# ciccio42/openvla-oft

Measured on AMD Instinct MI355X. Metric: fine-tune samples/s (action-chunks/s) OpenVLA-7B bf16, higher is better.
Workload: dtype bf16; 1 GPU; BASELINE.json configs[2]: LoRA r=32 fine-tune step (fwd+bwd+AdamW), 2x224x224 images + proprio, L1 head; global_batch=8, seq_len=608, parallelism=dp1, mask_mode=bidirectional

## Files before the change

### include/ovla.h

```cpp
#ifndef OVLA_H_
#define OVLA_H_

#include <stdint.h>

#ifdef __cplusplus
extern "C" {
#endif

#define OVLA_OK 0
#define OVLA_EINVAL (-1)
#define OVLA_EARCH (-2)
#define OVLA_ELAUNCH (-3)

#define OVLA_ABI_VERSION 1

const char* ovla_last_error(void);
int ovla_abi_version(void);
const char* ovla_build_hash(void);
int ovla_check_device(int device);

enum { OVLA_ACT_NONE = 0, OVLA_ACT_GELU = 1, OVLA_ACT_RELU = 2, OVLA_ACT_SILU = 3, OVLA_ACT_GELU_TANH = 4,
       OVLA_ACT_SWIGLU = 5 };

typedef struct {
  const void* A; int64_t lda;
  const void* B; int64_t ldb;
  const void* A2; int64_t lda2;
  const void* B2; int64_t ldb2;
  void* C; int64_t ldc;
  void* C_pre;
  const void* bias;
  const void* colscale;
  const void* residual; int64_t ldr;
  const void* film_gamma;
  const void* film_beta;
  int32_t film_rows;
  int32_t M, N, K, K2;
  int32_t k2_group_n;
  int32_t a_group_n;
  int32_t act;
  int32_t split_k;
  int32_t tile;
  float alpha;
  const void* dact_src; int64_t ld_dact;
  int32_t dact_mode, dact_act;
  const void* rope_cos; const void* rope_sin;
  int32_t rope_S, rope_cols;
  float* rowsq_out;
  const float* rowscale_part; int32_t rowscale_slots; float rowscale_eps; float* rowscale_r;
  uint32_t* hybrid_counters; int32_t n_hybrid_counters;
  void* workspace;
  int64_t workspace_bytes;
} ovla_gemm_args;

int ovla_gemm_plan(int32_t M, int32_t N, int32_t K, int32_t K2, int32_t k2_group_n, int64_t workspace_bytes, int32_t* tile,
                   int32_t* full_tiles, int32_t* rem_tiles, int32_t* rem_splits, double* est_seconds);
int ovla_gemm_resolved_tile(const ovla_gemm_args* a, int32_t* tile);
int64_t ovla_gemm_workspace_bytes(int32_t M, int32_t N, int32_t split_k);
int ovla_gemm_bf16(const ovla_gemm_args* a, void* stream);

typedef struct {
  int32_t tile;
  int32_t splits;
} ovla_gemm_schedule;
enum { OVLA_EPI_ROPE = 1,
       OVLA_EPI_ROWSCALE = 2,
       OVLA_EPI_SWIGLU = 4,
       OVLA_EPI_GENERAL = 8,
       OVLA_EPI_ROWSQ = 16     };
int ovla_gemm_fixed_schedule(int32_t N, int32_t K, int32_t K2, int32_t k2_group_n, int32_t epi_flags, ovla_gemm_schedule* out);
int64_t ovla_gemm_fixed_workspace_bytes(int32_t M, int32_t N, const ovla_gemm_schedule* s);
int ovla_gemm_bf16_fixed(const ovla_gemm_args* a, const ovla_gemm_schedule* s, void* stream);

typedef struct {
  const void* X; int64_t ldx;
  const void* Y; int64_t ldy;
  void* C; int64_t ldc;
  int32_t M, P, Q;
  float alpha;
  int32_t out_mode;
  float* W;
} ovla_gemm_tn_args;
int64_t ovla_gemm_tn_workspace_floats(const ovla_gemm_tn_args* a, int32_t group_size);
int ovla_gemm_tn_bf16(const ovla_gemm_tn_args* a, void* stream);
#define OVLA_TN_MAX_GROUP 4
int ovla_gemm_tn_grouped(const ovla_gemm_tn_args* problems, int32_t n, void* stream);

typedef struct {
  void* t; int64_t ld;
  const int32_t* obs_slot;
  const int32_t* obs_slot_host;
  int32_t M, G, n, r, rows_per_obs, n_obs;
} ovla_lora_route_args;
int ovla_lora_route(const ovla_lora_route_args* a, void* stream);

typedef struct {
  const void* src; void* dst;
  const int32_t* obs_slot; const int32_t* obs_slot_host;
  int64_t src_slot_stride;
  int32_t n, rows, dim, rows_per_obs, n_obs, elem_bytes;
} ovla_select_by_slot_args;
int ovla_select_by_slot(const ovla_select_by_slot_args* a, void* stream);

#define OVLA_MAX_SLOTS 4
#define OVLA_FILM_MAX_OBS 64
#define OVLA_FILM_ITEM_COLS 4
typedef struct { const void* W; const void* bias; void* out; int32_t out_f; int32_t item_start; } ovla_film_linear;
typedef struct {
  const void* table;
  const void* table_host;
  const void* avg; int64_t ld_avg;
  const int32_t* obs_slot;
  const int32_t* obs_slot_host;
  int32_t n_linears, n_obs, n, D;
} ovla_film_vectors_args;
int ovla_film_vectors(const ovla_film_vectors_args* a, void* stream);


typedef struct {
  const void* x; int64_t ldx;
  void* out[4];
  uint32_t module[4];
  uint32_t seed_lo, seed_hi, call;
  float p;
  int32_t M, K, G;
} ovla_lora_dropout_apply_args;
int ovla_lora_dropout_apply(const ovla_lora_dropout_apply_args* a, void* stream);

typedef struct {
  const void* x; int64_t ldx;
  const void* A; int64_t lda;
  void* t; int64_t ldt;
  uint32_t module[4];
  uint32_t seed_lo, seed_hi, call;
  float p, alpha;
  int32_t M, K, G, r;
} ovla_lora_dropout_proj_args;
int ovla_lora_dropout_proj(const ovla_lora_dropout_proj_args* a, void* stream);

typedef struct {
  void* dx; int64_t ld;
  const void* dt; int64_t ld_dt;
  const void* AT; int64_t ld_at;
  uint32_t module[4];
  uint32_t seed_lo, seed_hi, call;
  float p;
  int32_t M, K, G, r;
} ovla_lora_dropout_backproj_args;
int ovla_lora_dropout_backproj(const ovla_lora_dropout_backproj_args* a, void* stream);

typedef struct { const void* X; int64_t ldx; float* out; int32_t M, N; } ovla_colsum_args;
int ovla_colsum_bf16(const ovla_colsum_args* a, void* stream);

typedef struct {
  const void* Q; const void* K; const void* V; int64_t q_stride, k_stride, v_stride;
  void* O; int64_t o_stride;
  float* lse;
  const int32_t* kv_len;
  int32_t B, H, S, head_dim;
  int32_t causal;
  float scale;
} ovla_attn_fwd_args;
int ovla_attn_fwd(const ovla_attn_fwd_args* a, void* stream);

typedef struct {
  const void* Q; const void* K; const void* V; int64_t q_stride, k_stride, v_stride;
  const void* O; const void* dO; int64_t o_stride, do_stride;
  const float* lse;
  float* delta;
  void* dQ; void* dK; void* dV; int64_t dq_stride, dk_stride, dv_stride;
  const int32_t* kv_len;
  int32_t B, H, S, head_dim;
  int32_t causal;
  float scale;
  const void* rope_cos;
  const void* rope_sin;
} ovla_attn_bwd_args;
int ovla_attn_bwd(const ovla_attn_bwd_args* a, void* stream);

typedef struct {
  const void* Q; const void* K; int64_t q_stride, k_stride;
  const float* lse;
  const int32_t* kv_len;
  const int32_t* rows;
  float* P;
  float* P_mean;
  int32_t B, H, S, R, head_dim, causal; float scale;
} ovla_attn_probs_args;
int ovla_attn_probs(const ovla_attn_probs_args* a, void* stream);

typedef struct {
  const void* x; void* y; const void* weight; const void* bias;
  float* mean; float* rstd;
  int32_t rows, dim; float eps; int32_t is_rms;
} ovla_norm_fwd_args;
int ovla_norm_fwd(const ovla_norm_fwd_args* a, void* stream);

typedef struct {
  const void* x; const void* dy; const void* weight;
  const float* mean; const float* rstd;
  void* dx; float* dweight; float* dbias;
  int32_t rows, dim; int32_t is_rms; int32_t dx_accum;
} ovla_norm_bwd_args;
int ovla_norm_bwd(const ovla_norm_bwd_args* a, void* stream);

int ovla_rope_table(void* cos_table, void* sin_table, int32_t S, int32_t head_dim, float theta, void* stream);
typedef struct {
  void* qk; int64_t ld; int32_t rows, S, n_heads, head_dim;
  const void* cos_table; const void* sin_table; int32_t inverse;
} ovla_rope_args;
int ovla_rope(const ovla_rope_args* a, void* stream);

typedef struct { const void* gu; void* h; int32_t rows, F; } ovla_swiglu_fwd_args;
int ovla_swiglu_fwd(const ovla_swiglu_fwd_args* a, void* stream);
typedef struct { const void* gu; const void* dh; void* dgu; int32_t rows, F; } ovla_swiglu_bwd_args;
int ovla_swiglu_bwd(const ovla_swiglu_bwd_args* a, void* stream);

typedef struct { const void* z; const void* dh; void* dz; int64_t n; int32_t act; } ovla_act_bwd_args;
int ovla_act_bwd(const ovla_act_bwd_args* a, void* stream);

typedef struct { const void* a; const void* b; void* out; int64_t n; } ovla_add_args;
int ovla_add_bf16(const ovla_add_args* a, void* stream);
typedef struct { const void* x; const void* scale; void* out; int32_t rows, dim; } ovla_colscale_args;
int ovla_colscale_bf16(const ovla_colscale_args* a, void* stream);

typedef struct { const void* pixels; void* out; int64_t ldo; int32_t B, C_total, c0, H, W, patch, n_img, img_cstride; } ovla_im2col_args;
int ovla_im2col(const ovla_im2col_args* a, void* stream);

typedef struct { const void* src; void* dst; int32_t n_img, H, W, out, crop; float crop_scale; float mean[6]; float std[6]; } ovla_image_prep_args;
int ovla_image_prep(const ovla_image_prep_args* a, void* stream);

typedef struct {
  const void* src; void* dst; void* workspace; int64_t workspace_bytes;
  const int32_t* row_starts; const float* row_weights; const int32_t* col_starts; const float* col_weights;
  int32_t n_img, H, W, out_h, out_w, row_span, col_span;
} ovla_image_resize_args;
int64_t ovla_image_resize_workspace_bytes(int32_t n_img, int32_t W, int32_t out_h);
int ovla_image_resize(const ovla_image_resize_args* a, void* stream);

typedef struct { const void* src; void* dst; void* workspace; int64_t workspace_bytes; int32_t n_img, H, W, quality; } ovla_jpeg_roundtrip_args;
int64_t ovla_jpeg_roundtrip_workspace_bytes(int32_t n_img, int32_t H, int32_t W);
int ovla_jpeg_roundtrip(const ovla_jpeg_roundtrip_args* a, void* stream);

typedef struct {
  const void* src; void* dst; const float* params; void* workspace; int64_t workspace_bytes;
  int32_t n_img, H, W, out, ops_mask; float mean[6]; float std[6];
} ovla_image_augment_args;
int64_t ovla_image_augment_workspace_bytes(int32_t n_img, int32_t out);
int ovla_image_augment(const ovla_image_augment_args* a, void* stream);

typedef struct { const void* patches; const void* pos; const void* prefix; void* tokens; int32_t B, n_patches, n_prefix, dim; } ovla_vit_embed_args;
int ovla_vit_embed(const ovla_vit_embed_args* a, void* stream);
typedef struct {
  const void* src; void* dst; int32_t B, rows, dim;
  int64_t src_batch_stride, src_row0, src_ld, dst_batch_stride, dst_row0, dst_ld, dst_col0; int32_t accumulate;
} ovla_copy_rows_args;
int ovla_copy_rows(const ovla_copy_rows_args* a, void* stream);

typedef struct { void* dy; const void* x_pre; const void* gamma; float* dgamma; float* dbeta; int32_t B, rows_per_batch, dim; } ovla_film_bwd_args;
int ovla_film_bwd(const ovla_film_bwd_args* a, void* stream);

typedef struct { const void* x; const uint8_t* row_mask; void* out; int32_t B, L, dim; } ovla_masked_mean_args;
int ovla_masked_mean(const ovla_masked_mean_args* a, void* stream);

typedef struct { const int64_t* ids; const int64_t* labels; const void* embed_table; void* out; int32_t B, L, D, vocab; int64_t action_token_begin; } ovla_language_average_args;
int ovla_language_average(const ovla_language_average_args* a, void* stream);

typedef struct { const int64_t* ids; const int64_t* labels; const int32_t* lens; const void* embed_table; void* out; int32_t B, L, D, vocab; int64_t action_token_begin; } ovla_language_average_ragged_args;
int ovla_language_average_ragged(const ovla_language_average_ragged_args* a, void* stream);

typedef struct {
  const int64_t* ids; const int64_t* labels;
  const void* embed_table;
  const void* patches;
  const void* noisy;
  void* out;
  int32_t* action_pos;
  int32_t B, L, P, D, A, vocab;
  int32_t ignore_index, action_token_begin, action_dim;
} ovla_assemble_args;
int ovla_assemble_multimodal(const ovla_assemble_args* a, void* stream);

int ovla_row_sumsq(const void* x, int64_t ld, float* out, int32_t rows, int32_t dim, void* stream);

typedef struct { const void* src; const int32_t* index; void* dst; int32_t n, dim; int64_t src_ld, dst_ld; int32_t scatter_add; } ovla_gather_rows_args;
int ovla_gather_rows(const ovla_gather_rows_args* a, void* stream);

typedef struct {
  const void* logits; int64_t ld; const int64_t* targets; float* loss_rows; int32_t* argmax; void* dlogits; int64_t ld_d;
  int32_t rows, vocab; float grad_scale;
} ovla_token_ce_args;
int ovla_token_ce(const ovla_token_ce_args* a, void* stream);

typedef struct { const void* logits; int64_t ld; int32_t* token; int32_t* bin; int32_t rows, vocab, n_tokens, n_bins; } ovla_argmax_bins_args;
int ovla_argmax_bins(const ovla_argmax_bins_args* a, void* stream);

typedef struct {
  const void* x; const void* W; const void* b; void* pred;
  const void* target; float* loss_sum;
  int32_t rows, dim, adim;
  int32_t mse;
} ovla_head_out_fwd_args;
int ovla_head_out_fwd(const ovla_head_out_fwd_args* a, void* stream);
typedef struct {
  const void* x; const void* W; const void* pred; const void* target;
  const void* dpred;
  float dloss_scale;
  int32_t mse;
  void* dx; float* dW; float* db;
  int32_t rows, dim, adim;
} ovla_head_out_bwd_args;
int ovla_head_out_bwd(const ovla_head_out_bwd_args* a, void* stream);

typedef struct {
  void* param; void* exp_avg; void* exp_avg_sq;
  const float* grad;
  int64_t n; int32_t is_bf16; int32_t step;
  double lr, beta1, beta2, eps, weight_decay;
  float grad_scale;
} ovla_adamw_args;
int ovla_adamw(const ovla_adamw_args* a, void* stream);

typedef struct {
  const void* param;
  float* shadow;
  int64_t n; int32_t is_bf16;
  float one_minus_decay;
} ovla_ema_update_args;
int ovla_ema_update(const ovla_ema_update_args* a, void* stream);

#define OVLA_GRAD_SUMSQ_CHUNK 8192
#define OVLA_GRAD_SUMSQ_LANES 256
typedef struct {
  const float* grad;
  int64_t n; int32_t is_bf16;
  float grad_scale;
  double* slots; int32_t slot;
  double* workspace; int64_t workspace_bytes;
} ovla_grad_sumsq_args;
int ovla_grad_sumsq(const ovla_grad_sumsq_args* a, void* stream);

typedef struct { float coef; float norm; int32_t skip; int32_t n_steps, n_clipped, n_skipped; } ovla_grad_clip_state;
typedef struct {
  const double* slots; int32_t n_slots;
  float max_norm;
  int32_t skip_nonfinite;
  void* state;
} ovla_grad_clip_coef_args;
int ovla_grad_clip_coef(const ovla_grad_clip_coef_args* a, void* stream);

typedef struct {
  void* param; void* exp_avg; void* exp_avg_sq;
  const float* grad;
  int64_t n; int32_t is_bf16; int32_t step;
  double lr, beta1, beta2, eps, weight_decay;
  float grad_scale;
  const void* clip_state;
} ovla_adamw_clipped_args;
int ovla_adamw_clipped(const ovla_adamw_clipped_args* a, void* stream);

#define OVLA_TENSOR_STATS_PARTIAL_BYTES 32
typedef struct { int64_t offset, n; } ovla_tensor_seg;
typedef struct {
  double grad_sumsq, param_sumsq;
  float grad_absmax;
  int32_t n_bad_steps;
  int64_t n_nonfinite;
} ovla_tensor_stat;
int ovla_tensor_stats_plan(const ovla_tensor_seg* segs, int32_t n_segs, int64_t buffer_n, int32_t* chunk_start );
typedef struct {
  const float* grad;
  const void* param;
  int32_t param_is_bf16, grad_round_bf16;
  float grad_scale;
  const ovla_tensor_seg* segs;
  const int32_t* chunk_start;
  int32_t n_segs, total_chunks;
  void* partials;
  int64_t partials_bytes;
  ovla_tensor_stat* out;
} ovla_tensor_stats_args;
int ovla_tensor_stats(const ovla_tensor_stats_args* a, void* stream);

#define OVLA_ADAMW_MASTER_MAX_BLOCKS 2048
typedef struct {
  float* master; float* exp_avg; float* exp_avg_sq;
  void* param;
  const float* grad;
  int64_t n; int32_t step;
  double lr, beta1, beta2, eps, weight_decay;
  float grad_scale;
  const void* clip_state;
} ovla_adamw_master_args;
int ovla_adamw_master(const ovla_adamw_master_args* a, void* stream);

typedef struct { const int32_t* step; const void* temb_table; void* temb; const float* sample; void* noisy; int32_t n_steps, B, D, n; } ovla_ddim_prepare_args;
int ovla_ddim_prepare(const ovla_ddim_prepare_args* a, void* stream);
typedef struct { float* sample; const void* eps; const float* coef; int32_t* step; int32_t n_steps, n; } ovla_ddim_step_args;
int ovla_ddim_step(const ovla_ddim_step_args* a, void* stream);

typedef struct {
  const void* actions; int64_t ld_actions;
  const float* ab;
  const void* temb_table;
  void* noise; int64_t ld_noise;
  void* noisy; int64_t ld_noisy;
  void* temb; int64_t ld_temb;
  int32_t* timesteps;
  uint32_t seed_lo, seed_hi, call, stream;
  int32_t B, n, D, T;
} ovla_diffusion_noise_args;
int ovla_diffusion_noise(const ovla_diffusion_noise_args* a, void* stream);

#define OVLA_PG_GROUP_MAX 64
typedef struct {
  const void* logits; int64_t ld;
  int32_t* token; int32_t* bin; float* logprob; float* entropy;
  const uint32_t* state_dev; const int32_t* row_key;
  uint32_t seed_lo, seed_hi, call;
  float temperature;
  int32_t rows, vocab, lo, hi, n_tokens, n_bins, G;
} ovla_sample_tokens_group_args;
int ovla_sample_tokens_group(const ovla_sample_tokens_group_args* a, void* stream);

typedef struct {
  const void* logits; int64_t ld;
  const int32_t* tokens; const float* advantage; const float* old_logprob; const float* ref_logprob;
  float* logprob; float* ratio; int32_t* clipped; float* kl; float* entropy;
  void* dlogits; int64_t ld_d;
  float temperature, clip_lo, clip_hi, grad_scale, kl_coef, ent_scale;
  int32_t rows, G, vocab, lo, hi;
} ovla_token_pg_group_args;
int ovla_token_pg_group(const ovla_token_pg_group_args* a, void* stream);

typedef struct {
  const void* logits; int64_t ld;
  int32_t* token; int32_t* bin; float* logprob; float* entropy;
  const uint32_t* state_dev; const int32_t* row_key;
  uint32_t seed_lo, seed_hi, call;
  float temperature;
  int32_t rows, vocab, lo, hi, n_tokens, n_bins;
} ovla_sample_tokens_args;
int ovla_sample_tokens(const ovla_sample_tokens_args* a, void* stream);

typedef struct {
  const void* logits; int64_t ld;
  const int32_t* tokens; const float* advantage; const float* old_logprob;
  float* logprob; float* entropy; float* ratio; int32_t* clipped;
  void* dlogits; int64_t ld_d;
  float temperature, clip_lo, clip_hi, grad_scale;
  int32_t rows, vocab, lo, hi;
} ovla_token_pg_args;
int ovla_token_pg(const ovla_token_pg_args* a, void* stream);

typedef struct {
  const void* pred;
  float* action; float* logprob;
  const uint32_t* state_dev; const int32_t* row_key;
  uint32_t seed_lo, seed_hi, call;
  float scale[16], log_norm[16];
  int32_t rows, adim, G;
} ovla_laplace_sample_args;
int ovla_laplace_sample(const ovla_laplace_sample_args* a, void* stream);

typedef struct {
  const void* pred; const void* ref_pred;
  const float* actions; const float* advantage; const float* old_logprob;
  float* logprob; float* ratio; int32_t* clipped; float* kl;
  void* dpred;
  float scale[16], log_norm[16];
  float clip_lo, clip_hi, grad_scale, kl_coef, kl_scale;
  int32_t rows, adim, G;
} ovla_laplace_pg_args;
int ovla_laplace_pg(const ovla_laplace_pg_args* a, void* stream);

typedef struct {
  const void* pred; const void* log_scale;
  float* action; float* logprob; float* entropy;
  const uint32_t* state_dev; const int32_t* row_key;
  uint32_t seed_lo, seed_hi, call;
  float s_lo, s_hi;
  int32_t rows, adim, G;
} ovla_laplace_sample_rows_args;
int ovla_laplace_sample_rows(const ovla_laplace_sample_rows_args* a, void* stream);

typedef struct {
  const void* pred; const void* log_scale; const void* ref_pred; const void* ref_log_scale;
  const float* actions; const float* advantage; const float* old_logprob;
  float* logprob; float* ratio; int32_t* clipped; float* kl; float* entropy;
  void* dpred; void* dlog_scale;
  float s_lo, s_hi, clip_lo, clip_hi, grad_scale, kl_coef, kl_scale, entropy_coef, ent_scale;
  int32_t rows, adim, G;
} ovla_laplace_pg_rows_args;
int ovla_laplace_pg_rows(const ovla_laplace_pg_rows_args* a, void* stream);

typedef struct {
  const void* u; const float* returns; const float* old_value; const int32_t* valid;
  float* value; void* du; float* stats;
  float value_clip, grad_scale;
  int32_t B, chunk;
} ovla_value_loss_args;
int ovla_value_loss(const ovla_value_loss_args* a, void* stream);

typedef struct {
  const float* reward; const float* value; const float* bootstrap; const uint8_t* done;
  const int32_t* length; const int32_t* length_host;
  float* adv; float* ret;
  float gamma, gamma_lambda;
  int32_t N, T;
} ovla_gae_args;
int ovla_gae(const ovla_gae_args* a, void* stream);

typedef struct {
  float* adv; const int32_t* length; const int32_t* length_host;
  float eps;
  int32_t N, T;
} ovla_advantage_normalize_args;
int ovla_advantage_normalize(const ovla_advantage_normalize_args* a, void* stream);

typedef struct { const float* src; void* dst; int64_t n; float scale; } ovla_cvt_args;
int ovla_cvt_f32_to_bf16(const ovla_cvt_args* a, void* stream);
int ovla_cvt_bf16_to_f32(const void* src, float* dst, int64_t n, float scale, void* stream);

typedef struct { const void* src; void* dst; int32_t rows, cols; int64_t lds, ldd; } ovla_transpose_args;
int ovla_transpose_bf16(const ovla_transpose_args* a, void* stream);
int ovla_transpose_batched(const ovla_transpose_args* table, const int32_t* tile_start, int32_t n, int32_t total_tiles, void* stream);

typedef struct { const void* src; void* dst; int64_t src_ld_bytes, dst_ld_bytes, rows, row_bytes; } ovla_copy_entry;
int ovla_copy_table_plan(const ovla_copy_entry* entries, int32_t n, int32_t* tile_start);
int ovla_copy_table(const ovla_copy_entry* table, const int32_t* tile_start, int32_t n, int32_t total_tiles, void* stream);

int ovla_selftest_layouts(float* out, const void* src, void* stream);

#ifdef __cplusplus
}
#endif
#endif
```

### openvla-oft_amd/csrc/attention.hip

```cpp
#include "common.h"
#include <type_traits>

namespace {

constexpr int BQ = 64;
constexpr int BKV = 64;
constexpr float LOG2E = 1.4426950408889634f;
constexpr float LN2 = 0.6931471805599453f;

struct AttnParams {
  const bf16_bits *Q, *K, *V, *O, *dO;
  bf16_bits *Oout, *dQ, *dK, *dV;
  int64_t q_stride, k_stride, v_stride, o_stride, do_stride, dq_stride, dk_stride, dv_stride;
  float* lse;
  const float* lse_in;
  float* delta;
  const int32_t* kv_len;
  int B, H, S, hd, causal;
  float scale;
  const bf16_bits *rope_cos, *rope_sin;
  int xcd_map;
};

OVLA_DEV bf16x4_bits lds_tr16(const bf16_bits* p) {
  return __builtin_amdgcn_ds_read_tr16_b64_v4i16((__attribute__((address_space(3))) bf16x4_bits*)p);
}

OVLA_DEV bf16x8_bits tr_frag(const bf16_bits* tile, int row0, int col0, int stride, int lane) {
  const int g = lane >> 4, i = lane & 15;
  const bf16_bits* a0 = tile + (row0 + 4 * g + (i >> 2)) * stride + col0 + 4 * (i & 3);
  const bf16x4_bits lo = lds_tr16(a0);
  const bf16x4_bits hi = lds_tr16(a0 + 16 * stride);
  return bf16x8_bits{lo[0], lo[1], lo[2], lo[3], hi[0], hi[1], hi[2], hi[3]};
}

OVLA_DEV bf16x8_bits row_frag(const bf16_bits* tile, int row, int col0, int stride) {
  return *reinterpret_cast<const bf16x8_bits*>(tile + row * stride + col0);
}

OVLA_DEV bf16x8_bits zero8() { return bf16x8_bits{0, 0, 0, 0, 0, 0, 0, 0}; }

OVLA_DEV bf16x8_bits gload8(const bf16_bits* base, int64_t stride, int row, int col, int hd) {
  if (col >= hd) return zero8();
  return *reinterpret_cast<const bf16x8_bits*>(base + (int64_t)row * stride + col);
}

template <int DP>
OVLA_DEV bf16x8_bits gload8_nb(const bf16_bits* base, int64_t stride, int row, int col, int hd) {
  if constexpr (DP != 96) return *reinterpret_cast<const bf16x8_bits*>(base + (int64_t)row * stride + col);
  const bool in = col < hd;
  const bf16x8_bits v = *reinterpret_cast<const bf16x8_bits*>(base + (int64_t)row * stride + (in ? col : 0));
  return in ? v : zero8();
}

template <int DP, int NTHREADS = 256>
struct TileStage {
  static constexpr int CH = DP / 8;
  static constexpr int TOTAL = BKV * CH;
  static constexpr int PER_THREAD = (TOTAL + NTHREADS - 1) / NTHREADS;
  static constexpr int STRIDE = DP + 16;
  bf16x8_bits r[PER_THREAD];
  OVLA_DEV void load(const bf16_bits* base, int64_t stride, int row0, int row_last, int hd, int tid) {
#pragma unroll
    for (int i = 0; i < PER_THREAD; ++i) {
      const int id = tid + NTHREADS * i;
      const int rr = id / CH, ch = id % CH;
      int gr = row0 + rr;
      gr = gr < row_last ? gr : row_last;
      r[i] = (TOTAL % NTHREADS == 0 || id < TOTAL) ? gload8(base, stride, gr, ch * 8, hd) : zero8();
    }
  }
  OVLA_DEV void store(bf16_bits* tile, int tid) const {
#pragma unroll
    for (int i = 0; i < PER_THREAD; ++i) {
      const int id = tid + NTHREADS * i;
      const int rr = id / CH, ch = id % CH;
      if (TOTAL % NTHREADS == 0 || id < TOTAL) *reinterpret_cast<bf16x8_bits*>(tile + rr * STRIDE + ch * 8) = r[i];
    }
  }
};

OVLA_DEV short f2bf_s(float f) { return (short)f2bf(f); }

OVLA_DEV int xcd_contiguous(int n, int total) {
  const int per = total >> 3;
  return n < 8 * per ? (n & 7) * per + (n >> 3) : n;
}

template <int DP, int NW>
__global__ __launch_bounds__(64 * NW) void attn_fwd_kernel(const AttnParams p) {
  constexpr int KS = DP / 32;
  constexpr int DT = DP / 16;
  constexpr int STRIDE = DP + 16;
  constexpr int NTH = 64 * NW;
  constexpr int BQW = 16 * NW;
  __shared__ __attribute__((aligned(16))) bf16_bits Ks[2][BKV * STRIDE];
  __shared__ __attribute__((aligned(16))) bf16_bits Vs[2][BKV * STRIDE];

  const int tid = threadIdx.x, lane = tid & 63, wave = tid >> 6, g = lane >> 4;
  const int b = blockIdx.z, h = blockIdx.y, q0 = blockIdx.x * BQW;
  const int qrow = q0 + wave * 16 + (lane & 15);
  const int qrow_c = qrow < p.S ? qrow : p.S - 1;
  const int kvlen = p.kv_len ? p.kv_len[b] : p.S;
  int kv_end = kvlen < p.S ? kvlen : p.S;
  if (p.causal) kv_end = kv_end < (q0 + BQW) ? kv_end : (q0 + BQW);
  const int ntiles = (kv_end + BKV - 1) / BKV;

  const bf16_bits* Qb = p.Q + (int64_t)b * p.S * p.q_stride + (int64_t)h * p.hd;
  const bf16_bits* Kb = p.K + (int64_t)b * p.S * p.k_stride + (int64_t)h * p.hd;
  const bf16_bits* Vb = p.V + (int64_t)b * p.S * p.v_stride + (int64_t)h * p.hd;

  bf16x8_bits qf[KS];
#pragma unroll
  for (int s = 0; s < KS; ++s) qf[s] = gload8(Qb, p.q_stride, qrow_c, 32 * s + 8 * g, p.hd);

  f32x4 accO[DT];
#pragma unroll
  for (int d = 0; d < DT; ++d) accO[d] = f32x4{0.f, 0.f, 0.f, 0.f};
  float m_run = -INFINITY, l_run = 0.f;
  const float sl2 = p.scale * LOG2E;

  TileStage<DP, NTH> kst, vst;
  if (ntiles > 0) {
    kst.load(Kb, p.k_stride, 0, p.S - 1, p.hd, tid);
    vst.load(Vb, p.v_stride, 0, p.S - 1, p.hd, tid);
    kst.store(Ks[0], tid);
    vst.store(Vs[0], tid);
    if (ntiles > 1) {
      kst.load(Kb, p.k_stride, BKV, p.S - 1, p.hd, tid);
      vst.load(Vb, p.v_stride, BKV, p.S - 1, p.hd, tid);
    }
  }
  __syncthreads();

  auto tile = [&](int t, auto mask_tag) {
    constexpr bool MASK = decltype(mask_tag)::value;
    const bf16_bits* Kt = Ks[t & 1];
    const bf16_bits* Vt = Vs[t & 1];
    f32x4 accS[4];
#pragma unroll
    for (int nt = 0; nt < 4; ++nt) {
      accS[nt] = f32x4{0.f, 0.f, 0.f, 0.f};
#pragma unroll
      for (int s = 0; s < KS; ++s)
        accS[nt] = __builtin_amdgcn_mfma_f32_16x16x32_bf16(row_frag(Kt, nt * 16 + (lane & 15), 32 * s + 8 * g, STRIDE), qf[s],
                                                           accS[nt], 0, 0, 0);
    }
    const int kbase = t * BKV;
    float mx = -INFINITY;
#pragma unroll
    for (int nt = 0; nt < 4; ++nt)
#pragma unroll
      for (int j = 0; j < 4; ++j) {
        float sv = accS[nt][j] * sl2;
        if constexpr (MASK) {
          const int key = kbase + nt * 16 + 4 * g + j;
          const bool ok = key < kvlen && (!p.causal || key <= qrow);
          sv = ok ? sv : -INFINITY;
        }
        accS[nt][j] = sv;
        mx = fmaxf(mx, sv);
      }
    mx = fmaxf(mx, __shfl_xor(mx, 16, 64));
    mx = fmaxf(mx, __shfl_xor(mx, 32, 64));
    const float m_new = fmaxf(m_run, mx);
    const float m_safe = (m_new == -INFINITY) ? 0.f : m_new;
    const float alpha = __builtin_amdgcn_exp2f(m_run - m_safe);
    float psum = 0.f;
#pragma unroll
    for (int nt = 0; nt < 4; ++nt)
#pragma unroll
      for (int j = 0; j < 4; ++j) {
        const float pv = __builtin_amdgcn_exp2f(accS[nt][j] - m_safe);
        accS[nt][j] = pv;
        psum += pv;
      }
    l_run = l_run * alpha + psum;
    m_run = m_new;
#pragma unroll
    for (int d = 0; d < DT; ++d)
#pragma unroll
      for (int j = 0; j < 4; ++j) accO[d][j] *= alpha;
#pragma unroll
    for (int s2 = 0; s2 < 2; ++s2) {
      bf16x8_bits pf;
#pragma unroll
      for (int j = 0; j < 4; ++j) {
        pf[j] = f2bf_s(accS[2 * s2][j]);
        pf[4 + j] = f2bf_s(accS[2 * s2 + 1][j]);
      }
#pragma unroll
      for (int d = 0; d < DT; ++d)
        accO[d] = __builtin_amdgcn_mfma_f32_16x16x32_bf16(tr_frag(Vt, 32 * s2, d * 16, STRIDE, lane), pf, accO[d], 0, 0, 0);
    }
    if (t + 1 < ntiles) {
      kst.store(Ks[(t + 1) & 1], tid);
      vst.store(Vs[(t + 1) & 1], tid);
      if (t + 2 < ntiles) {
        kst.load(Kb, p.k_stride, (t + 2) * BKV, p.S - 1, p.hd, tid);
        vst.load(Vb, p.v_stride, (t + 2) * BKV, p.S - 1, p.hd, tid);
      }
    }
    __syncthreads();
  };
  int n_free = kvlen / BKV;
  if (p.causal) n_free = n_free < (q0 / BKV) ? n_free : (q0 / BKV);
  if (n_free > ntiles) n_free = ntiles;
  for (int t = 0; t < n_free; ++t) tile(t, std::false_type{});
  for (int t = n_free; t < ntiles; ++t) tile(t, std::true_type{});
  l_run += __shfl_xor(l_run, 16, 64);
  l_run += __shfl_xor(l_run, 32, 64);
  const float inv_l = l_run > 0.f ? 1.0f / l_run : 0.f;
  if (qrow < p.S) {
    bf16_bits* Ob = p.Oout + ((int64_t)b * p.S + qrow) * p.o_stride + (int64_t)h * p.hd;
#pragma unroll
    for (int d = 0; d < DT; ++d) {
      const int col = d * 16 + 4 * g;
      if (col < p.hd) {
        bf16x4_bits o;
#pragma unroll
        for (int j = 0; j < 4; ++j) o[j] = f2bf_s(accO[d][j] * inv_l);
        *reinterpret_cast<bf16x4_bits*>(Ob + col) = o;
      }
    }
    if (g == 0 && p.lse) p.lse[((int64_t)b * p.H + h) * p.S + qrow] = m_run * LN2 + __logf(l_run);
  }
}

typedef __attribute__((ext_vector_type(16))) float f32x16;

template <int DP> struct Fwd32Cfg {
  static constexpr int KSTR = DP + 8;
  static constexpr int VSTR = (DP == 96) ? DP : DP + 32;
};

template <int DP, int STRIDE, int NTHREADS>
struct TileStageS {
  static constexpr int CH = DP / 8;
  static constexpr int TOTAL = BKV * CH;
  static_assert(TOTAL % NTHREADS == 0, "tile chunks must divide over the workgroup");
  static constexpr int PER_THREAD = TOTAL / NTHREADS;
  bf16x8_bits r[PER_THREAD];
  OVLA_DEV void load(const bf16_bits* base, int64_t stride, int row0, int row_last, int hd, int tid) {
#pragma unroll
    for (int i = 0; i < PER_THREAD; ++i) {
      const int id = tid + NTHREADS * i;
      const int rr = id / CH, ch = id % CH;
      int gr = row0 + rr;
      gr = gr < row_last ? gr : row_last;
      r[i] = gload8_nb<DP>(base, stride, gr, ch * 8, hd);
    }
  }
  OVLA_DEV void store(bf16_bits* tile, int tid) const {
#pragma unroll
    for (int i = 0; i < PER_THREAD; ++i) {
      const int id = tid + NTHREADS * i;
      const int rr = id / CH, ch = id % CH;
      *reinterpret_cast<bf16x8_bits*>(tile + rr * STRIDE + ch * 8) = r[i];
    }
  }
};

OVLA_DEV bf16x8_bits tr_frag32(const bf16_bits* tile, int row0, int col0, int stride, int lane) {
  const int h = lane >> 5, g4 = (lane >> 4) & 1, i = lane & 15;
  const bf16_bits* a0 = tile + (row0 + 4 * h + (i >> 2)) * stride + col0 + 16 * g4 + 4 * (i & 3);
  const bf16x4_bits lo = lds_tr16(a0);
  const bf16x4_bits hi = lds_tr16(a0 + 8 * stride);
  return bf16x8_bits{lo[0], lo[1], lo[2], lo[3], hi[0], hi[1], hi[2], hi[3]};
}

template <int DP>
__global__ __launch_bounds__(256, 2) void attn_fwd32_kernel(const AttnParams p) {
  constexpr int KS = DP / 16;
  constexpr int DB = DP / 32;
  constexpr int KSTR = Fwd32Cfg<DP>::KSTR, VSTR = Fwd32Cfg<DP>::VSTR;
  constexpr int BQW = 128;
  __shared__ __attribute__((aligned(16))) bf16_bits Ks[2][BKV * KSTR];
  __shared__ __attribute__((aligned(16))) bf16_bits Vs[2][BKV * VSTR];

  const int tid = threadIdx.x, lane = tid & 63, wave = tid >> 6, hi = lane >> 5;
  const int nqb = (p.S + BQW - 1) / BQW;
  const int wi = p.xcd_map ? xcd_contiguous(blockIdx.x, gridDim.x) : blockIdx.x;
  const int bh = wi / nqb, b = bh / p.H, h = bh - b * p.H, q0 = (wi - bh * nqb) * BQW;
  const int qrow = q0 + wave * 32 + (lane & 31);
  const int qrow_c = qrow < p.S ? qrow : p.S - 1;
  const int kvlen = p.kv_len ? p.kv_len[b] : p.S;
  int kv_end = kvlen < p.S ? kvlen : p.S;
  if (p.causal) kv_end = kv_end < (q0 + BQW) ? kv_end : (q0 + BQW);
  const int ntiles = (kv_end + BKV - 1) / BKV;

  const bf16_bits* Qb = p.Q + (int64_t)b * p.S * p.q_stride + (int64_t)h * p.hd;
  const bf16_bits* Kb = p.K + (int64_t)b * p.S * p.k_stride + (int64_t)h * p.hd;
  const bf16_bits* Vb = p.V + (int64_t)b * p.S * p.v_stride + (int64_t)h * p.hd;

  bf16x8_bits qf[KS];
#pragma unroll
  for (int s = 0; s < KS; ++s) qf[s] = gload8_nb<DP>(Qb, p.q_stride, qrow_c, 16 * s + 8 * hi, p.hd);

  f32x16 accO[DB];
#pragma unroll
  for (int d = 0; d < DB; ++d)
#pragma unroll
    for (int r = 0; r < 16; ++r) accO[d][r] = 0.f;
  float m_run = -INFINITY, l_run = 0.f;
  const float sl2 = p.scale * LOG2E;

  TileStageS<DP, KSTR, 256> kst;
  TileStageS<DP, VSTR, 256> vst;
  if (ntiles > 0) {
    kst.load(Kb, p.k_stride, 0, p.S - 1, p.hd, tid);
    vst.load(Vb, p.v_stride, 0, p.S - 1, p.hd, tid);
    kst.store(Ks[0], tid);
    vst.store(Vs[0], tid);
  }
  __syncthreads();

  auto tile = [&](int t, auto mask_tag) {
    constexpr bool MASK = decltype(mask_tag)::value;
    const bf16_bits* Kt = Ks[t & 1];
    const bf16_bits* Vt = Vs[t & 1];
    kst.load(Kb, p.k_stride, (t + 1) * BKV, p.S - 1, p.hd, tid);
    vst.load(Vb, p.v_stride, (t + 1) * BKV, p.S - 1, p.hd, tid);
    f32x16 accS[2];
#pragma unroll
    for (int kb = 0; kb < 2; ++kb)
#pragma unroll
      for (int r = 0; r < 16; ++r) accS[kb][r] = 0.f;
    {
      constexpr int HS = KS / 2;
      const bf16_bits* krow = Kt + (lane & 31) * KSTR + 8 * hi;
      bf16x8_bits ka[HS], kb_[HS];
#pragma unroll
      for (int s = 0; s < HS; ++s) ka[s] = *reinterpret_cast<const bf16x8_bits*>(krow + 16 * s);
#pragma unroll
      for (int s = 0; s < HS; ++s) kb_[s] = *reinterpret_cast<const bf16x8_bits*>(krow + 16 * (HS + s));
      __builtin_amdgcn_sched_barrier(0);
#pragma unroll
      for (int s = 0; s < HS; ++s) accS[0] = __builtin_amdgcn_mfma_f32_32x32x16_bf16(ka[s], qf[s], accS[0], 0, 0, 0);
      __builtin_amdgcn_sched_barrier(0);
#pragma unroll
      for (int s = 0; s < HS; ++s) ka[s] = *reinterpret_cast<const bf16x8_bits*>(krow + 32 * KSTR + 16 * s);
      __builtin_amdgcn_sched_barrier(0);
#pragma unroll
      for (int s = 0; s < HS; ++s) accS[0] = __builtin_amdgcn_mfma_f32_32x32x16_bf16(kb_[s], qf[HS + s], accS[0], 0, 0, 0);
      __builtin_amdgcn_sched_barrier(0);
#pragma unroll
      for (int s = 0; s < HS; ++s) kb_[s] = *reinterpret_cast<const bf16x8_bits*>(krow + 32 * KSTR + 16 * (HS + s));
      __builtin_amdgcn_sched_barrier(0);
#pragma unroll
      for (int s = 0; s < HS; ++s) accS[1] = __builtin_amdgcn_mfma_f32_32x32x16_bf16(ka[s], qf[s], accS[1], 0, 0, 0);
#pragma unroll
      for (int s = 0; s < HS; ++s) accS[1] = __builtin_amdgcn_mfma_f32_32x32x16_bf16(kb_[s], qf[HS + s], accS[1], 0, 0, 0);
    }
    const int kbase = t * BKV;
    float mx = -INFINITY;
#pragma unroll
    for (int kb = 0; kb < 2; ++kb)
#pragma unroll
      for (int r = 0; r < 16; ++r) {
        if constexpr (MASK) {
          const int key = kbase + kb * 32 + (r & 3) + 8 * (r >> 2) + 4 * hi;
          const bool ok = key < kvlen && (!p.causal || key <= qrow);
          accS[kb][r] = ok ? accS[kb][r] : -INFINITY;
        }
        mx = fmaxf(mx, accS[kb][r]);
      }
    mx = fmaxf(mx, __shfl_xor(mx, 32, 64));
    const float m_new = fmaxf(m_run, mx);
    const float m_safe = (m_new == -INFINITY) ? 0.f : m_new;
    const float alpha = __builtin_amdgcn_exp2f((m_run - m_safe) * sl2);
    const float moff = -m_safe * sl2;
    float psum = 0.f;
#pragma unroll
    for (int kb = 0; kb < 2; ++kb)
#pragma unroll
      for (int r = 0; r < 16; ++r) {
        const float pv = __builtin_amdgcn_exp2f(__builtin_fmaf(accS[kb][r], sl2, moff));
        accS[kb][r] = pv;
        psum += pv;
      }
    l_run = l_run * alpha + psum;
    m_run = m_new;
#pragma unroll
    for (int d = 0; d < DB; ++d)
#pragma unroll
      for (int r = 0; r < 16; ++r) accO[d][r] *= alpha;
#pragma unroll
    for (int kb = 0; kb < 2; ++kb)
#pragma unroll
      for (int tt = 0; tt < 2; ++tt) {
        bf16x8_bits pf;
#pragma unroll
        for (int j = 0; j < 8; ++j) pf[j] = f2bf_s(accS[kb][8 * tt + j]);
#pragma unroll
        for (int d = 0; d < DB; ++d)
          accO[d] = __builtin_amdgcn_mfma_f32_32x32x16_bf16(tr_frag32(Vt, kb * 32 + 16 * tt, d * 32, VSTR, lane), pf, accO[d], 0, 0, 0);
      }
    kst.store(Ks[(t + 1) & 1], tid);
    vst.store(Vs[(t + 1) & 1], tid);
    __syncthreads();
  };
  int n_free = kvlen / BKV;
  if (p.causal) n_free = n_free < (q0 / BKV) ? n_free : (q0 / BKV);
  if (n_free > ntiles) n_free = ntiles;
  for (int t = 0; t < n_free; ++t) tile(t, std::false_type{});
  for (int t = n_free; t < ntiles; ++t) tile(t, std::true_type{});
  l_run += __shfl_xor(l_run, 32, 64);
  const float inv_l = l_run > 0.f ? 1.0f / l_run : 0.f;
  if (qrow < p.S) {
    bf16_bits* Ob = p.Oout + ((int64_t)b * p.S + qrow) * p.o_stride + (int64_t)h * p.hd;
#pragma unroll
    for (int d = 0; d < DB; ++d)
#pragma unroll
      for (int rq = 0; rq < 4; ++rq) {
        const int col = d * 32 + 8 * rq + 4 * hi;
        if (col < p.hd) {
          bf16x4_bits o;
#pragma unroll
          for (int j = 0; j < 4; ++j) o[j] = f2bf_s(accO[d][4 * rq + j] * inv_l);
          *reinterpret_cast<bf16x4_bits*>(Ob + col) = o;
        }
      }
    if (hi == 0 && p.lse) p.lse[((int64_t)b * p.H + h) * p.S + qrow] = m_run * sl2 * LN2 + __logf(l_run);
  }
}

template <int DT>
OVLA_DEV void inverse_rope_store(const f32x4 (&acc)[DT], float scale, bf16_bits* dst, int hd, int pos, int g, const bf16_bits* cosT, const bf16_bits* sinT) {
  constexpr int HT = DT / 2;
  const int half = hd >> 1;
#pragma unroll
  for (int d = 0; d < HT; ++d) {
    const int col = d * 16 + 4 * g;
    const bf16x4_bits cs = *reinterpret_cast<const bf16x4_bits*>(cosT + (int64_t)pos * half + col);
    const bf16x4_bits sn = *reinterpret_cast<const bf16x4_bits*>(sinT + (int64_t)pos * half + col);
    bf16x4_bits olo, ohi;
#pragma unroll
    for (int j = 0; j < 4; ++j) {
      const float a = bfround(acc[d][j] * scale), b = bfround(acc[d + HT][j] * scale);
      const float cc = bf2f((bf16_bits)cs[j]), s = -bf2f((bf16_bits)sn[j]);
      olo[j] = (short)f2bf(bfround(a * cc) + bfround(-b * s));
      ohi[j] = (short)f2bf(bfround(b * cc) + bfround(a * s));
    }
    *reinterpret_cast<bf16x4_bits*>(dst + col) = olo;
    *reinterpret_cast<bf16x4_bits*>(dst + half + col) = ohi;
  }
}

template <int DP, int NW, int OCC = 2, bool BATCH = (DP == 128)>
__global__ __launch_bounds__(64 * NW, OCC) void attn_bwd_dq_kernel(const AttnParams p) {
  constexpr int KS = DP / 32, DT = DP / 16, STRIDE = DP + 16;
  constexpr int NTH = 64 * NW;
  constexpr int BQW = 16 * NW;
  __shared__ __attribute__((aligned(16))) bf16_bits Ks[2][BKV * STRIDE];
  __shared__ __attribute__((aligned(16))) bf16_bits Vs[2][BKV * STRIDE];
  const int tid = threadIdx.x, lane = tid & 63, wave = tid >> 6, g = lane >> 4;
  int b = blockIdx.z, h = blockIdx.y, q0 = blockIdx.x * BQW;
  if (p.xcd_map) {
    const int nqb = (p.S + BQW - 1) / BQW;
    const int wi = xcd_contiguous(blockIdx.x, gridDim.x), bh = wi / nqb;
    b = bh / p.H; h = bh - b * p.H; q0 = (wi - bh * nqb) * BQW;
  }
  const int qrow = q0 + wave * 16 + (lane & 15);
  const int qrow_c = qrow < p.S ? qrow : p.S - 1;
  const int kvlen = p.kv_len ? p.kv_len[b] : p.S;
  int kv_end = kvlen < p.S ? kvlen : p.S;
  if (p.causal) kv_end = kv_end < (q0 + BQW) ? kv_end : (q0 + BQW);
  const int ntiles = (kv_end + BKV - 1) / BKV;

  const bf16_bits* Qb = p.Q + (int64_t)b * p.S * p.q_stride + (int64_t)h * p.hd;
  const bf16_bits* Kb = p.K + (int64_t)b * p.S * p.k_stride + (int64_t)h * p.hd;
  const bf16_bits* Vb = p.V + (int64_t)b * p.S * p.v_stride + (int64_t)h * p.hd;
  const bf16_bits* dOb = p.dO + (int64_t)b * p.S * p.do_stride + (int64_t)h * p.hd;

  bf16x8_bits qf[KS], dof[KS];
#pragma unroll
  for (int s = 0; s < KS; ++s) {
    qf[s] = gload8(Qb, p.q_stride, qrow_c, 32 * s + 8 * g, p.hd);
    dof[s] = gload8(dOb, p.do_stride, qrow_c, 32 * s + 8 * g, p.hd);
  }
  const int64_t stat = ((int64_t)b * p.H + h) * p.S + qrow_c;
  const float Lq = p.lse_in[stat] * LOG2E;
  float Dq = 0.f;
  {
    const bf16_bits* Ob = p.O + (int64_t)b * p.S * p.o_stride + (int64_t)h * p.hd;
#pragma unroll
    for (int s = 0; s < KS; ++s) {
      const bf16x8_bits of = gload8(Ob, p.o_stride, qrow_c, 32 * s + 8 * g, p.hd);
#pragma unroll
      for (int j = 0; j < 8; ++j) Dq += bf2f((bf16_bits)of[j]) * bf2f((bf16_bits)dof[s][j]);
    }
    Dq += __shfl_xor(Dq, 16, 64);
    Dq += __shfl_xor(Dq, 32, 64);
    if (g == 0 && qrow < p.S) p.delta[stat] = Dq;
  }
  const float sl2 = p.scale * LOG2E;

  f32x4 accQ[DT];
#pragma unroll
  for (int d = 0; d < DT; ++d) accQ[d] = f32x4{0.f, 0.f, 0.f, 0.f};

  TileStage<DP, NTH> kst, vst;
  if (ntiles > 0) {
    kst.load(Kb, p.k_stride, 0, p.S - 1, p.hd, tid);
    vst.load(Vb, p.v_stride, 0, p.S - 1, p.hd, tid);
    kst.store(Ks[0], tid);
    vst.store(Vs[0], tid);
    if (ntiles > 1) {
      kst.load(Kb, p.k_stride, BKV, p.S - 1, p.hd, tid);
      vst.load(Vb, p.v_stride, BKV, p.S - 1, p.hd, tid);
    }
  }
  __syncthreads();
  auto tile = [&](int t, auto mask_tag) {
    constexpr bool MASK = decltype(mask_tag)::value;
    const bf16_bits* Kt = Ks[t & 1];
    const bf16_bits* Vt = Vs[t & 1];
    const int kbase = t * BKV;
#pragma unroll
    for (int s2 = 0; s2 < 2; ++s2) {
      f32x4 accS[2], accP[2];
      if constexpr (BATCH) {
        bf16x8_bits kfr[2][KS], vfr[2][KS];
#pragma unroll
        for (int nn = 0; nn < 2; ++nn)
#pragma unroll
          for (int s = 0; s < KS; ++s) {
            kfr[nn][s] = row_frag(Kt, (2 * s2 + nn) * 16 + (lane & 15), 32 * s + 8 * g, STRIDE);
            vfr[nn][s] = row_frag(Vt, (2 * s2 + nn) * 16 + (lane & 15), 32 * s + 8 * g, STRIDE);
          }
        __builtin_amdgcn_sched_barrier(0);
#pragma unroll
        for (int nn = 0; nn < 2; ++nn) {
          accS[nn] = f32x4{0.f, 0.f, 0.f, 0.f};
          accP[nn] = f32x4{0.f, 0.f, 0.f, 0.f};
        }
#pragma unroll
        for (int s = 0; s < KS; ++s)
#pragma unroll
          for (int nn = 0; nn < 2; ++nn) {
            accS[nn] = __builtin_amdgcn_mfma_f32_16x16x32_bf16(kfr[nn][s], qf[s], accS[nn], 0, 0, 0);
            accP[nn] = __builtin_amdgcn_mfma_f32_16x16x32_bf16(vfr[nn][s], dof[s], accP[nn], 0, 0, 0);
          }
        __builtin_amdgcn_sched_barrier(0);
      } else {
#pragma unroll
      for (int nn = 0; nn < 2; ++nn) {
        const int nt = 2 * s2 + nn;
        accS[nn] = f32x4{0.f, 0.f, 0.f, 0.f};
        accP[nn] = f32x4{0.f, 0.f, 0.f, 0.f};
#pragma unroll
        for (int s = 0; s < KS; ++s) {
          accS[nn] = __builtin_amdgcn_mfma_f32_16x16x32_bf16(row_frag(Kt, nt * 16 + (lane & 15), 32 * s + 8 * g, STRIDE), qf[s], accS[nn], 0, 0, 0);
          accP[nn] = __builtin_amdgcn_mfma_f32_16x16x32_bf16(row_frag(Vt, nt * 16 + (lane & 15), 32 * s + 8 * g, STRIDE), dof[s], accP[nn], 0, 0, 0);
        }
      }
      }
      bf16x8_bits dsf;
#pragma unroll
      for (int nn = 0; nn < 2; ++nn)
#pragma unroll
        for (int j = 0; j < 4; ++j) {
          float pv = __builtin_amdgcn_exp2f(accS[nn][j] * sl2 - Lq);
          if constexpr (MASK) {
            const int key = kbase + (2 * s2 + nn) * 16 + 4 * g + j;
            const bool ok = key < kvlen && (!p.causal || key <= qrow);
            pv = ok ? pv : 0.f;
          }
          dsf[4 * nn + j] = f2bf_s(pv * (accP[nn][j] - Dq));
        }
      if constexpr (BATCH) {
        bf16x8_bits ktr[DT];
#pragma unroll
        for (int d = 0; d < DT; ++d) ktr[d] = tr_frag(Kt, 32 * s2, d * 16, STRIDE, lane);
        __builtin_amdgcn_sched_barrier(0);
#pragma unroll
        for (int d = 0; d < DT; ++d) accQ[d] = __builtin_amdgcn_mfma_f32_16x16x32_bf16(ktr[d], dsf, accQ[d], 0, 0, 0);
      } else {
#pragma unroll
      for (int d = 0; d < DT; ++d)
        accQ[d] = __builtin_amdgcn_mfma_f32_16x16x32_bf16(tr_frag(Kt, 32 * s2, d * 16, STRIDE, lane), dsf, accQ[d], 0, 0, 0);
      }
    }
    if (t + 1 < ntiles) {
      kst.store(Ks[(t + 1) & 1], tid);
      vst.store(Vs[(t + 1) & 1], tid);
      if (t + 2 < ntiles) {
        kst.load(Kb, p.k_stride, (t + 2) * BKV, p.S - 1, p.hd, tid);
        vst.load(Vb, p.v_stride, (t + 2) * BKV, p.S - 1, p.hd, tid);
      }
    }
    __syncthreads();
  };
  int n_free = kvlen / BKV;
  if (p.causal) n_free = n_free < (q0 / BKV) ? n_free : (q0 / BKV);
  if (n_free > ntiles) n_free = ntiles;
  for (int t = 0; t < n_free; ++t) tile(t, std::false_type{});
  for (int t = n_free; t < ntiles; ++t) tile(t, std::true_type{});
  if (qrow < p.S) {
    bf16_bits* dQb = p.dQ + ((int64_t)b * p.S + qrow) * p.dq_stride + (int64_t)h * p.hd;
    if (p.rope_cos) {
      inverse_rope_store<DT>(accQ, p.scale, dQb, p.hd, qrow, g, p.rope_cos, p.rope_sin);
    } else {
#pragma unroll
      for (int d = 0; d < DT; ++d) {
        const int col = d * 16 + 4 * g;
        if (col < p.hd) {
          bf16x4_bits o;
#pragma unroll
          for (int j = 0; j < 4; ++j) o[j] = f2bf_s(accQ[d][j] * p.scale);
          *reinterpret_cast<bf16x4_bits*>(dQb + col) = o;
        }
      }
    }
  }
}


template <int DP, int NW>
__global__ __launch_bounds__(64 * NW, 2) void attn_bwd_dkv_kernel(const AttnParams p) {
  constexpr int KS = DP / 32, DT = DP / 16, STRIDE = DP + 16;
  constexpr int NTH = 64 * NW;
  constexpr int BKW = 16 * NW;
  __shared__ __attribute__((aligned(16))) bf16_bits Qs[2][BQ * STRIDE];
  __shared__ __attribute__((aligned(16))) bf16_bits dOs[2][BQ * STRIDE];
  __shared__ float Ls[2][BQ], Ds[2][BQ];
  const int tid = threadIdx.x, lane = tid & 63, wave = tid >> 6, g = lane >> 4;
  int b = blockIdx.z, h = blockIdx.y, k0 = blockIdx.x * BKW;
  if (p.xcd_map) {
    const int nkb = (p.S + BKW - 1) / BKW;
    const int wi = xcd_contiguous(blockIdx.x, gridDim.x), bh = wi / nkb;
    b = bh / p.H; h = bh - b * p.H; k0 = (wi - bh * nkb) * BKW;
  }
  const int krow = k0 + wave * 16 + (lane & 15);
  const int krow_c = krow < p.S ? krow : p.S - 1;
  const int kvlen = p.kv_len ? p.kv_len[b] : p.S;

  const bf16_bits* Qb = p.Q + (int64_t)b * p.S * p.q_stride + (int64_t)h * p.hd;
  const bf16_bits* Kb = p.K + (int64_t)b * p.S * p.k_stride + (int64_t)h * p.hd;
  const bf16_bits* Vb = p.V + (int64_t)b * p.S * p.v_stride + (int64_t)h * p.hd;
  const bf16_bits* dOb = p.dO + (int64_t)b * p.S * p.do_stride + (int64_t)h * p.hd;
  const float* lse_b = p.lse_in + ((int64_t)b * p.H + h) * p.S;
  const float* del_b = p.delta + ((int64_t)b * p.H + h) * p.S;

  bf16x8_bits kf[KS], vf[KS];
#pragma unroll
  for (int s = 0; s < KS; ++s) {
    kf[s] = gload8(Kb, p.k_stride, krow_c, 32 * s + 8 * g, p.hd);
    vf[s] = gload8(Vb, p.v_stride, krow_c, 32 * s + 8 * g, p.hd);
  }
  const float sl2 = p.scale * LOG2E;
  f32x4 accK[DT], accV[DT];
#pragma unroll
  for (int d = 0; d < DT; ++d) {
    accK[d] = f32x4{0.f, 0.f, 0.f, 0.f};
    accV[d] = f32x4{0.f, 0.f, 0.f, 0.f};
  }
  const bool key_ok = krow < kvlen && krow < p.S;
  const int nq = (p.S + BQ - 1) / BQ;
  const int qt0 = p.causal ? (k0 / BQ) : 0;

  TileStage<DP, NTH> qst, dst;
  float lreg = 0.f, dreg = 0.f;
  auto load_tile = [&](int qt) {
    qst.load(Qb, p.q_stride, qt * BQ, p.S - 1, p.hd, tid);
    dst.load(dOb, p.do_stride, qt * BQ, p.S - 1, p.hd, tid);
    if (tid < BQ) {
      int r = qt * BQ + tid;
      r = r < p.S ? r : p.S - 1;
      lreg = lse_b[r] * LOG2E;
      dreg = del_b[r];
    }
  };
  auto store_tile = [&](int buf) {
    qst.store(Qs[buf], tid);
    dst.store(dOs[buf], tid);
    if (tid < BQ) {
      Ls[buf][tid] = lreg;
      Ds[buf][tid] = dreg;
    }
  };
  if (qt0 < nq) {
    load_tile(qt0);
    store_tile(0);
    if (qt0 + 1 < nq) load_tile(qt0 + 1);
  }
  __syncthreads();

  auto tile = [&](int qt, auto mask_tag) {
    constexpr bool MASK = decltype(mask_tag)::value;
    const int buf = (qt - qt0) & 1;
    const bf16_bits* Qt = Qs[buf];
    const bf16_bits* dOt = dOs[buf];
    const float* Lt = Ls[buf];
    const float* Dt = Ds[buf];
    const int qbase = qt * BQ;
#pragma unroll
    for (int s2 = 0; s2 < 2; ++s2) {
      f32x4 accS[2], accP[2];
#pragma unroll
      for (int mm = 0; mm < 2; ++mm) {
        const int mt = 2 * s2 + mm;
        accS[mm] = f32x4{0.f, 0.f, 0.f, 0.f};
        accP[mm] = f32x4{0.f, 0.f, 0.f, 0.f};
#pragma unroll
        for (int s = 0; s < KS; ++s) {
          accS[mm] = __builtin_amdgcn_mfma_f32_16x16x32_bf16(row_frag(Qt, mt * 16 + (lane & 15), 32 * s + 8 * g, STRIDE), kf[s], accS[mm], 0, 0, 0);
          accP[mm] = __builtin_amdgcn_mfma_f32_16x16x32_bf16(row_frag(dOt, mt * 16 + (lane & 15), 32 * s + 8 * g, STRIDE), vf[s], accP[mm], 0, 0, 0);
        }
      }
#pragma unroll
      for (int mm = 0; mm < 2; ++mm)
#pragma unroll
        for (int j = 0; j < 4; ++j) {
          const int ql = (2 * s2 + mm) * 16 + 4 * g + j;
          float pv = __builtin_amdgcn_exp2f(accS[mm][j] * sl2 - Lt[ql]);
          if constexpr (MASK) {
            const int q = qbase + ql;
            const bool ok = key_ok && q < p.S && (!p.causal || krow <= q);
            pv = ok ? pv : 0.f;
          }
          accS[mm][j] = pv;
          accP[mm][j] = pv * (accP[mm][j] - Dt[ql]);
        }
      bf16x8_bits pf, dsf;
#pragma unroll
      for (int j = 0; j < 4; ++j) {
        pf[j] = f2bf_s(accS[0][j]);
        pf[4 + j] = f2bf_s(accS[1][j]);
        dsf[j] = f2bf_s(accP[0][j]);
        dsf[4 + j] = f2bf_s(accP[1][j]);
      }
#pragma unroll
      for (int d = 0; d < DT; ++d) {
        accV[d] = __builtin_amdgcn_mfma_f32_16x16x32_bf16(tr_frag(dOt, 32 * s2, d * 16, STRIDE, lane), pf, accV[d], 0, 0, 0);
        accK[d] = __builtin_amdgcn_mfma_f32_16x16x32_bf16(tr_frag(Qt, 32 * s2, d * 16, STRIDE, lane), dsf, accK[d], 0, 0, 0);
      }
    }
    if (qt + 1 < nq) {
      store_tile(buf ^ 1);
      if (qt + 2 < nq) load_tile(qt + 2);
    }
    __syncthreads();
  };
  const bool keys_full = k0 + BKW <= kvlen && k0 + BKW <= p.S;
  for (int qt = qt0; qt < nq; ++qt) {
    const bool free_tile = keys_full && (qt + 1) * BQ <= p.S && (!p.causal || qt * BQ >= k0 + BKW - 1);
    if (free_tile) tile(qt, std::false_type{});
    else tile(qt, std::true_type{});
  }
  if (krow < p.S) {
    bf16_bits* dKb = p.dK + ((int64_t)b * p.S + krow) * p.dk_stride + (int64_t)h * p.hd;
    bf16_bits* dVb = p.dV + ((int64_t)b * p.S + krow) * p.dv_stride + (int64_t)h * p.hd;
    if (p.rope_cos) inverse_rope_store<DT>(accK, p.scale, dKb, p.hd, krow, g, p.rope_cos, p.rope_sin);
#pragma unroll
    for (int d = 0; d < DT; ++d) {
      const int col = d * 16 + 4 * g;
      if (col < p.hd) {
        bf16x4_bits ok_, ov_;
#pragma unroll
        for (int j = 0; j < 4; ++j) {
          ok_[j] = f2bf_s(accK[d][j] * p.scale);
          ov_[j] = f2bf_s(accV[d][j]);
        }
        if (!p.rope_cos) *reinterpret_cast<bf16x4_bits*>(dKb + col) = ok_;
        *reinterpret_cast<bf16x4_bits*>(dVb + col) = ov_;
      }
    }
  }
}

int check_common(int B, int H, int S, int hd, const char* who) {
  if (!(B > 0 && H > 0 && S > 0)) {
    ovla_set_error("%s: empty problem B=%d H=%d S=%d", who, B, H, S);
    return OVLA_EINVAL;
  }
  if (!(hd == 64 || hd == 72 || hd == 128)) {
    ovla_set_error("%s: head_dim %d not supported (64, 72, 128)", who, hd);
    return OVLA_EINVAL;
  }
  return OVLA_OK;
}

inline bool stride_ok(int64_t s) { return (s % 8) == 0; }

}

extern "C" int ovla_attn_fwd(const ovla_attn_fwd_args* a, void* stream_) {
  hipStream_t stream = (hipStream_t)stream_;
  OVLA_REQUIRE(a && a->Q && a->K && a->V && a->O, "ovla_attn_fwd: null pointer");
  if (int rc = check_common(a->B, a->H, a->S, a->head_dim, "ovla_attn_fwd")) return rc;
  OVLA_REQUIRE(stride_ok(a->q_stride) && stride_ok(a->k_stride) && stride_ok(a->v_stride) && (a->o_stride % 4) == 0,
               "ovla_attn_fwd: row strides must be multiples of 8 elements");
  OVLA_REQUIRE(aligned16(a->Q) && aligned16(a->K) && aligned16(a->V) && (((uintptr_t)a->O) & 7) == 0, "ovla_attn_fwd: alignment");
  AttnParams p = {};
  p.Q = (const bf16_bits*)a->Q; p.K = (const bf16_bits*)a->K; p.V = (const bf16_bits*)a->V; p.Oout = (bf16_bits*)a->O;
  p.q_stride = a->q_stride; p.k_stride = a->k_stride; p.v_stride = a->v_stride; p.o_stride = a->o_stride;
  p.lse = a->lse; p.kv_len = a->kv_len; p.B = a->B; p.H = a->H; p.S = a->S; p.hd = a->head_dim; p.causal = a->causal; p.scale = a->scale;
  static const bool fwd32 = []() { const char* e = getenv("OVLA_ATTN_FWD32"); return !(e && e[0] == '0'); }();
  static const bool xcd_map = []() { const char* e = getenv("OVLA_ATTN_XCD"); return !(e && e[0] == '0'); }();
  p.xcd_map = xcd_map ? 1 : 0;
  if (fwd32 && a->S > 64) {
    const dim3 grid((unsigned)(cdiv(a->S, 128) * a->H * a->B));
    switch (a->head_dim) {
      case 64: hipLaunchKernelGGL((attn_fwd32_kernel<64>), grid, dim3(256), 0, stream, p); break;
      case 72: hipLaunchKernelGGL((attn_fwd32_kernel<96>), grid, dim3(256), 0, stream, p); break;
      default: hipLaunchKernelGGL((attn_fwd32_kernel<128>), grid, dim3(256), 0, stream, p); break;
    }
  } else if (a->S > 64) {
    const dim3 grid(cdiv(a->S, 128), a->H, a->B);
    switch (a->head_dim) {
      case 64: hipLaunchKernelGGL((attn_fwd_kernel<64, 8>), grid, dim3(512), 0, stream, p); break;
      case 72: hipLaunchKernelGGL((attn_fwd_kernel<96, 8>), grid, dim3(512), 0, stream, p); break;
      default: hipLaunchKernelGGL((attn_fwd_kernel<128, 8>), grid, dim3(512), 0, stream, p); break;
    }
  } else {
    const dim3 grid(cdiv(a->S, BQ), a->H, a->B);
    switch (a->head_dim) {
      case 64: hipLaunchKernelGGL((attn_fwd_kernel<64, 4>), grid, dim3(256), 0, stream, p); break;
      case 72: hipLaunchKernelGGL((attn_fwd_kernel<96, 4>), grid, dim3(256), 0, stream, p); break;
      default: hipLaunchKernelGGL((attn_fwd_kernel<128, 4>), grid, dim3(256), 0, stream, p); break;
    }
  }
  OVLA_CHECK_LAUNCH("ovla_attn_fwd");
  return OVLA_OK;
}

extern "C" int ovla_attn_bwd(const ovla_attn_bwd_args* a, void* stream_) {
  hipStream_t stream = (hipStream_t)stream_;
  OVLA_REQUIRE(a && a->Q && a->K && a->V && a->O && a->dO && a->lse && a->delta && a->dQ && a->dK && a->dV, "ovla_attn_bwd: null pointer");
  if (int rc = check_common(a->B, a->H, a->S, a->head_dim, "ovla_attn_bwd")) return rc;
  OVLA_REQUIRE(stride_ok(a->q_stride) && stride_ok(a->k_stride) && stride_ok(a->v_stride) && stride_ok(a->o_stride) && stride_ok(a->do_stride) &&
                   (a->dq_stride % 4) == 0 && (a->dk_stride % 4) == 0 && (a->dv_stride % 4) == 0,
               "ovla_attn_bwd: row strides must be multiples of 8 elements");
  OVLA_REQUIRE(aligned16(a->Q) && aligned16(a->K) && aligned16(a->V) && aligned16(a->O) && aligned16(a->dO), "ovla_attn_bwd: alignment");
  if (a->rope_cos || a->rope_sin)
    OVLA_REQUIRE(a->rope_cos && a->rope_sin && (a->head_dim == 128 || a->head_dim == 64) && (((uintptr_t)a->rope_cos | (uintptr_t)a->rope_sin) & 7) == 0,
                 "ovla_attn_bwd: fused inverse RoPE needs both tables (8-byte aligned) and head_dim 64 or 128");
  AttnParams p = {};
  p.Q = (const bf16_bits*)a->Q; p.K = (const bf16_bits*)a->K; p.V = (const bf16_bits*)a->V; p.O = (const bf16_bits*)a->O;
  p.dO = (const bf16_bits*)a->dO; p.dQ = (bf16_bits*)a->dQ; p.dK = (bf16_bits*)a->dK; p.dV = (bf16_bits*)a->dV;
  p.q_stride = a->q_stride; p.k_stride = a->k_stride; p.v_stride = a->v_stride; p.o_stride = a->o_stride; p.do_stride = a->do_stride;
  p.dq_stride = a->dq_stride; p.dk_stride = a->dk_stride; p.dv_stride = a->dv_stride;
  p.lse_in = a->lse; p.delta = a->delta; p.kv_len = a->kv_len;
  p.B = a->B; p.H = a->H; p.S = a->S; p.hd = a->head_dim; p.causal = a->causal; p.scale = a->scale;
  p.rope_cos = (const bf16_bits*)a->rope_cos; p.rope_sin = (const bf16_bits*)a->rope_sin;
  static const bool xcd_map = []() { const char* e = getenv("OVLA_ATTN_XCD"); return !(e && e[0] == '0'); }();
  p.xcd_map = xcd_map ? 1 : 0;
  const dim3 grid = xcd_map ? dim3((unsigned)(cdiv(a->S, BQ) * a->H * a->B)) : dim3(cdiv(a->S, BQ), a->H, a->B);
  const dim3 grid_kv4 = grid;
  const dim3 grid_kv8 = xcd_map ? dim3((unsigned)(cdiv(a->S, 128) * a->H * a->B)) : dim3(cdiv(a->S, 128), a->H, a->B);
  switch (a->head_dim) {
    case 64:
      hipLaunchKernelGGL((attn_bwd_dq_kernel<64, 4>), grid, dim3(256), 0, stream, p);
      hipLaunchKernelGGL((attn_bwd_dkv_kernel<64, 4>), grid_kv4, dim3(256), 0, stream, p);
      break;
    case 72:
      if (a->S % 128 == 0 || a->S > 512) {
        hipLaunchKernelGGL((attn_bwd_dq_kernel<96, 8>), grid_kv8, dim3(512), 0, stream, p);
        hipLaunchKernelGGL((attn_bwd_dkv_kernel<96, 8>), grid_kv8, dim3(512), 0, stream, p);
      } else {
        hipLaunchKernelGGL((attn_bwd_dq_kernel<96, 4>), grid, dim3(256), 0, stream, p);
        hipLaunchKernelGGL((attn_bwd_dkv_kernel<96, 4>), grid_kv4, dim3(256), 0, stream, p);
      }
      break;
    default:
      {
        static const bool dq_batch = []() { const char* e = getenv("OVLA_ATTN_DQ_BATCH"); return !(e && e[0] == '0'); }();
        if (dq_batch) hipLaunchKernelGGL((attn_bwd_dq_kernel<128, 8>), grid_kv8, dim3(512), 0, stream, p);
        else hipLaunchKernelGGL((attn_bwd_dq_kernel<128, 8, 2, false>), grid_kv8, dim3(512), 0, stream, p);
      }
      hipLaunchKernelGGL((attn_bwd_dkv_kernel<128, 8>), grid_kv8, dim3(512), 0, stream, p);
      break;
  }
  OVLA_CHECK_LAUNCH("ovla_attn_bwd");
  return OVLA_OK;
}
```

Baseline: 49.34 samples/s.

## Add LDS-resident whole-sequence attention kernels for small-head vision encoders

Adds forward and backward attention kernels that stage a (batch, head) pair's entire K/V (or Q/dO for dK/dV) into up to 160KB of dynamic LDS, with one workgroup per batch-head. Waves then loop over query or key row tasks against the resident tiles. The path is used for head_dim 64/72 with unmasked, non-causal sequences up to an LDS-derived length, once batch*heads passes per-shape thresholds. The goal is to cut redundant global K/V reloads and launch count, since backward fuses dQ and dK/dV into one kernel. The cost is lower occupancy from the heavy LDS use and less grid parallelism, because there is one block per batch-head.

```diff
diff --git a/include/ovla.h b/include/ovla.h
--- a/include/ovla.h
+++ b/include/ovla.h
@@ -178,6 +178,11 @@
 } ovla_attn_bwd_args;
 int ovla_attn_bwd(const ovla_attn_bwd_args* a, void* stream);
 
+int64_t ovla_attn_resident_lds_bytes(int32_t head_dim, int32_t S, int32_t backward);
+int32_t ovla_attn_resident_max_s(int32_t head_dim);
+int32_t ovla_attn_resident_min_bh(int32_t head_dim, int32_t backward);
+int64_t ovla_attn_resident_launches(void);
+
 typedef struct {
   const void* Q; const void* K; int64_t q_stride, k_stride;
   const float* lse;
diff --git a/openvla-oft_amd/csrc/attention.hip b/openvla-oft_amd/csrc/attention.hip
--- a/openvla-oft_amd/csrc/attention.hip
+++ b/openvla-oft_amd/csrc/attention.hip
@@ -1,4 +1,7 @@
 #include "common.h"
+#include <atomic>
+#include <cstdint>
+#include <cstdlib>
 #include <type_traits>
 
 namespace {
@@ -269,6 +272,111 @@
   return bf16x8_bits{lo[0], lo[1], lo[2], lo[3], hi[0], hi[1], hi[2], hi[3]};
 }
 
+template <int DP, bool MASK>
+OVLA_DEV void fwd32_tile_math(const bf16_bits* Kt, const bf16_bits* Vt, const bf16x8_bits (&qf)[DP / 16], f32x16 (&accO)[DP / 32], float& m_run, float& l_run,
+                             int kbase, int kvlen, int causal, int qrow, float sl2, int lane) {
+  constexpr int KS = DP / 16, DB = DP / 32;
+  constexpr int KSTR = Fwd32Cfg<DP>::KSTR, VSTR = Fwd32Cfg<DP>::VSTR;
+  const int hi = lane >> 5;
+  f32x16 accS[2];
+#pragma unroll
+  for (int kb = 0; kb < 2; ++kb)
+#pragma unroll
+    for (int r = 0; r < 16; ++r) accS[kb][r] = 0.f;
+  {
+    constexpr int HS = KS / 2;
+    const bf16_bits* krow = Kt + (lane & 31) * KSTR + 8 * hi;
+    bf16x8_bits ka[HS], kb_[HS];
+#pragma unroll
+    for (int s = 0; s < HS; ++s) ka[s] = *reinterpret_cast<const bf16x8_bits*>(krow + 16 * s);
+#pragma unroll
+    for (int s = 0; s < HS; ++s) kb_[s] = *reinterpret_cast<const bf16x8_bits*>(krow + 16 * (HS + s));
+    __builtin_amdgcn_sched_barrier(0);
+#pragma unroll
+    for (int s = 0; s < HS; ++s) accS[0] = __builtin_amdgcn_mfma_f32_32x32x16_bf16(ka[s], qf[s], accS[0], 0, 0, 0);
+    __builtin_amdgcn_sched_barrier(0);
+#pragma unroll
+    for (int s = 0; s < HS; ++s) ka[s] = *reinterpret_cast<const bf16x8_bits*>(krow + 32 * KSTR + 16 * s);
+    __builtin_amdgcn_sched_barrier(0);
+#pragma unroll
+    for (int s = 0; s < HS; ++s) accS[0] = __builtin_amdgcn_mfma_f32_32x32x16_bf16(kb_[s], qf[HS + s], accS[0], 0, 0, 0);
+    __builtin_amdgcn_sched_barrier(0);
+#pragma unroll
+    for (int s = 0; s < HS; ++s) kb_[s] = *reinterpret_cast<const bf16x8_bits*>(krow + 32 * KSTR + 16 * (HS + s));
+    __builtin_amdgcn_sched_barrier(0);
+#pragma unroll
+    for (int s = 0; s < HS; ++s) accS[1] = __builtin_amdgcn_mfma_f32_32x32x16_bf16(ka[s], qf[s], accS[1], 0, 0, 0);
+#pragma unroll
+    for (int s = 0; s < HS; ++s) accS[1] = __builtin_amdgcn_mfma_f32_32x32x16_bf16(kb_[s], qf[HS + s], accS[1], 0, 0, 0);
+  }
+  float mx = -INFINITY;
+#pragma unroll
+  for (int kb = 0; kb < 2; ++kb)
+#pragma unroll
+    for (int r = 0; r < 16; ++r) {
+      if constexpr (MASK) {
+        const int key = kbase + kb * 32 + (r & 3) + 8 * (r >> 2) + 4 * hi;
+        const bool ok = key < kvlen && (!causal || key <= qrow);
+        accS[kb][r] = ok ? accS[kb][r] : -INFINITY;
+      }
+      mx = fmaxf(mx, accS[kb][r]);
+    }
+  mx = fmaxf(mx, __shfl_xor(mx, 32, 64));
+  const float m_new = fmaxf(m_run, mx);
+  const float m_safe = (m_new == -INFINITY) ? 0.f : m_new;
+  const float alpha = __builtin_amdgcn_exp2f((m_run - m_safe) * sl2);
+  const float moff = -m_safe * sl2;
+  float psum = 0.f;
+#pragma unroll
+  for (int kb = 0; kb < 2; ++kb)
+#pragma unroll
+    for (int r = 0; r < 16; ++r) {
+      const float pv = __builtin_amdgcn_exp2f(__builtin_fmaf(accS[kb][r], sl2, moff));
+      accS[kb][r] = pv;
+      psum += pv;
+    }
+  l_run = l_run * alpha + psum;
+  m_run = m_new;
+#pragma unroll
+  for (int d = 0; d < DB; ++d)
+#pragma unroll
+    for (int r = 0; r < 16; ++r) accO[d][r] *= alpha;
+#pragma unroll
+  for (int kb = 0; kb < 2; ++kb)
+#pragma unroll
+    for (int tt = 0; tt < 2; ++tt) {
+      bf16x8_bits pf;
+#pragma unroll
+      for (int j = 0; j < 8; ++j) pf[j] = f2bf_s(accS[kb][8 * tt + j]);
+#pragma unroll
+      for (int d = 0; d < DB; ++d)
+        accO[d] = __builtin_amdgcn_mfma_f32_32x32x16_bf16(tr_frag32(Vt, kb * 32 + 16 * tt, d * 32, VSTR, lane), pf, accO[d], 0, 0, 0);
+    }
+}
+
+template <int DP>
+OVLA_DEV void fwd32_finish(const AttnParams& p, const f32x16 (&accO)[DP / 32], float m_run, float l_run, int b, int h, int qrow, float sl2, int hi) {
+  constexpr int DB = DP / 32;
+  l_run += __shfl_xor(l_run, 32, 64);
+  const float inv_l = l_run > 0.f ? 1.0f / l_run : 0.f;
+  if (qrow < p.S) {
+    bf16_bits* Ob = p.Oout + ((int64_t)b * p.S + qrow) * p.o_stride + (int64_t)h * p.hd;
+#pragma unroll
+    for (int d = 0; d < DB; ++d)
+#pragma unroll
+      for (int rq = 0; rq < 4; ++rq) {
+        const int col = d * 32 + 8 * rq + 4 * hi;
+        if (col < p.hd) {
+          bf16x4_bits o;
+#pragma unroll
+          for (int j = 0; j < 4; ++j) o[j] = f2bf_s(accO[d][4 * rq + j] * inv_l);
+          *reinterpret_cast<bf16x4_bits*>(Ob + col) = o;
+        }
+      }
+    if (hi == 0 && p.lse) p.lse[((int64_t)b * p.H + h) * p.S + qrow] = m_run * sl2 * LN2 + __logf(l_run);
+  }
+}
+
 template <int DP>
 __global__ __launch_bounds__(256, 2) void attn_fwd32_kernel(const AttnParams p) {
   constexpr int KS = DP / 16;
@@ -321,81 +429,7 @@
     const bf16_bits* Vt = Vs[t & 1];
     kst.load(Kb, p.k_stride, (t + 1) * BKV, p.S - 1, p.hd, tid);
     vst.load(Vb, p.v_stride, (t + 1) * BKV, p.S - 1, p.hd, tid);
-    f32x16 accS[2];
-#pragma unroll
-    for (int kb = 0; kb < 2; ++kb)
-#pragma unroll
-      for (int r = 0; r < 16; ++r) accS[kb][r] = 0.f;
-    {
-      constexpr int HS = KS / 2;
-      const bf16_bits* krow = Kt + (lane & 31) * KSTR + 8 * hi;
-      bf16x8_bits ka[HS], kb_[HS];
-#pragma unroll
-      for (int s = 0; s < HS; ++s) ka[s] = *reinterpret_cast<const bf16x8_bits*>(krow + 16 * s);
-#pragma unroll
-      for (int s = 0; s < HS; ++s) kb_[s] = *reinterpret_cast<const bf16x8_bits*>(krow + 16 * (HS + s));
-      __builtin_amdgcn_sched_barrier(0);
-#pragma unroll
-      for (int s = 0; s < HS; ++s) accS[0] = __builtin_amdgcn_mfma_f32_32x32x16_bf16(ka[s], qf[s], accS[0], 0, 0, 0);
-      __builtin_amdgcn_sched_barrier(0);
-#pragma unroll
-      for (int s = 0; s < HS; ++s) ka[s] = *reinterpret_cast<const bf16x8_bits*>(krow + 32 * KSTR + 16 * s);
-      __builtin_amdgcn_sched_barrier(0);
-#pragma unroll
-      for (int s = 0; s < HS; ++s) accS[0] = __builtin_amdgcn_mfma_f32_32x32x16_bf16(kb_[s], qf[HS + s], accS[0], 0, 0, 0);
-      __builtin_amdgcn_sched_barrier(0);
-#pragma unroll
-      for (int s = 0; s < HS; ++s) kb_[s] = *reinterpret_cast<const bf16x8_bits*>(krow + 32 * KSTR + 16 * (HS + s));
-      __builtin_amdgcn_sched_barrier(0);
-#pragma unroll
-      for (int s = 0; s < HS; ++s) accS[1] = __builtin_amdgcn_mfma_f32_32x32x16_bf16(ka[s], qf[s], accS[1], 0, 0, 0);
-#pragma unroll
-      for (int s = 0; s < HS; ++s) accS[1] = __builtin_amdgcn_mfma_f32_32x32x16_bf16(kb_[s], qf[HS + s], accS[1], 0, 0, 0);
-    }
-    const int kbase = t * BKV;
-    float mx = -INFINITY;
-#pragma unroll
-    for (int kb = 0; kb < 2; ++kb)
-#pragma unroll
-      for (int r = 0; r < 16; ++r) {
-        if constexpr (MASK) {
-          const int key = kbase + kb * 32 + (r & 3) + 8 * (r >> 2) + 4 * hi;
-          const bool ok = key < kvlen && (!p.causal || key <= qrow);
-          accS[kb][r] = ok ? accS[kb][r] : -INFINITY;
-        }
-        mx = fmaxf(mx, accS[kb][r]);
-      }
-    mx = fmaxf(mx, __shfl_xor(mx, 32, 64));
-    const float m_new = fmaxf(m_run, mx);
-    const float m_safe = (m_new == -INFINITY) ? 0.f : m_new;
-    const float alpha = __builtin_amdgcn_exp2f((m_run - m_safe) * sl2);
-    const float moff = -m_safe * sl2;
-    float psum = 0.f;
-#pragma unroll
-    for (int kb = 0; kb < 2; ++kb)
-#pragma unroll
-      for (int r = 0; r < 16; ++r) {
-        const float pv = __builtin_amdgcn_exp2f(__builtin_fmaf(accS[kb][r], sl2, moff));
-        accS[kb][r] = pv;
-        psum += pv;
-      }
-    l_run = l_run * alpha + psum;
-    m_run = m_new;
-#pragma unroll
-    for (int d = 0; d < DB; ++d)
-#pragma unroll
-      for (int r = 0; r < 16; ++r) accO[d][r] *= alpha;
-#pragma unroll
-    for (int kb = 0; kb < 2; ++kb)
-#pragma unroll
-      for (int tt = 0; tt < 2; ++tt) {
-        bf16x8_bits pf;
-#pragma unroll
-        for (int j = 0; j < 8; ++j) pf[j] = f2bf_s(accS[kb][8 * tt + j]);
-#pragma unroll
-        for (int d = 0; d < DB; ++d)
-          accO[d] = __builtin_amdgcn_mfma_f32_32x32x16_bf16(tr_frag32(Vt, kb * 32 + 16 * tt, d * 32, VSTR, lane), pf, accO[d], 0, 0, 0);
-      }
+    fwd32_tile_math<DP, MASK>(Kt, Vt, qf, accO, m_run, l_run, t * BKV, kvlen, p.causal, qrow, sl2, lane);
     kst.store(Ks[(t + 1) & 1], tid);
     vst.store(Vs[(t + 1) & 1], tid);
     __syncthreads();
@@ -405,23 +439,89 @@
   if (n_free > ntiles) n_free = ntiles;
   for (int t = 0; t < n_free; ++t) tile(t, std::false_type{});
   for (int t = n_free; t < ntiles; ++t) tile(t, std::true_type{});
-  l_run += __shfl_xor(l_run, 32, 64);
-  const float inv_l = l_run > 0.f ? 1.0f / l_run : 0.f;
-  if (qrow < p.S) {
-    bf16_bits* Ob = p.Oout + ((int64_t)b * p.S + qrow) * p.o_stride + (int64_t)h * p.hd;
+  fwd32_finish<DP>(p, accO, m_run, l_run, b, h, qrow, sl2, hi);
+}
+
+constexpr int RES_LDS_BYTES = 160 * 1024;
+
+constexpr int res_dp(int hd) { return hd == 64 ? 64 : 96; }
+inline int64_t resident_lds_bytes(int hd, int S, bool backward) {
+  const int64_t rows = (int64_t)cdiv(S, BKV) * BKV, dp = res_dp(hd);
+  if (backward) return rows * (2 * (dp + 16) * 2 + 2 * 4);
+  return rows * 2 * ((dp + 8) + (dp == 96 ? dp : dp + 32));
+}
+inline int resident_max_s(int hd) {
+  if (!(hd == 64 || hd == 72)) return 0;
+  int tiles = 0;
+  while (resident_lds_bytes(hd, (tiles + 1) * BKV, false) <= RES_LDS_BYTES && resident_lds_bytes(hd, (tiles + 1) * BKV, true) <= RES_LDS_BYTES) ++tiles;
+  return tiles * BKV;
+}
+
+template <int DP, int STRIDE>
+OVLA_DEV void stage_resident(bf16_bits* dst, const bf16_bits* base, int64_t stride, int ntiles, int row_last, int hd, int tid, int nthreads) {
+  constexpr int CH = DP / 8;
+  const int total = ntiles * BKV * CH;
+  for (int id0 = tid; id0 < total; id0 += 4 * nthreads) {
+    bf16x8_bits r[4];
+#pragma unroll
+    for (int i = 0; i < 4; ++i) {
+      const int id = id0 + i * nthreads;
+      const int idc = id < total ? id : total - 1;
+      const int rr = idc / CH, ch = idc % CH;
+      r[i] = gload8_nb<DP>(base, stride, rr < row_last ? rr : row_last, ch * 8, hd);
+    }
+#pragma unroll
+    for (int i = 0; i < 4; ++i) {
+      const int id = id0 + i * nthreads;
+      if (id < total) *reinterpret_cast<bf16x8_bits*>(dst + (id / CH) * STRIDE + (id % CH) * 8) = r[i];
+    }
+  }
+}
+
+template <int DP, int NWMAX>
+__global__ __launch_bounds__(64 * NWMAX) void attn_fwd_resident_kernel(const AttnParams p) {
+  constexpr int KS = DP / 16, DB = DP / 32;
+  constexpr int KSTR = Fwd32Cfg<DP>::KSTR, VSTR = Fwd32Cfg<DP>::VSTR;
+  extern __shared__ __attribute__((aligned(16))) char res_smem[];
+  const int ntiles = (p.S + BKV - 1) / BKV;
+  bf16_bits* Ks = reinterpret_cast<bf16_bits*>(res_smem);
+  bf16_bits* Vs = Ks + ntiles * BKV * KSTR;
+
+  const int tid = threadIdx.x, lane = tid & 63, wave = tid >> 6, hi = lane >> 5, nwaves = blockDim.x >> 6;
+  const int bh = blockIdx.x, b = bh / p.H, h = bh - b * p.H;
+  const bf16_bits* Qb = p.Q + (int64_t)b * p.S * p.q_stride + (int64_t)h * p.hd;
+  const bf16_bits* Kb = p.K + (int64_t)b * p.S * p.k_stride + (int64_t)h * p.hd;
+  const bf16_bits* Vb = p.V + (int64_t)b * p.S * p.v_stride + (int64_t)h * p.hd;
+  const float sl2 = p.scale * LOG2E;
+  const int ntasks = (p.S + 31) / 32, n_free = p.S / BKV;
+
+  int qrow = wave * 32 + (lane & 31);
+  int qrow_c = qrow < p.S ? qrow : p.S - 1;
+  bf16x8_bits qf[KS];
+#pragma unroll
+  for (int s = 0; s < KS; ++s) qf[s] = gload8_nb<DP>(Qb, p.q_stride, qrow_c, 16 * s + 8 * hi, p.hd);
+  stage_resident<DP, KSTR>(Ks, Kb, p.k_stride, ntiles, p.S - 1, p.hd, tid, blockDim.x);
+  stage_resident<DP, VSTR>(Vs, Vb, p.v_stride, ntiles, p.S - 1, p.hd, tid, blockDim.x);
+  __syncthreads();
+
+  for (int task = wave; task < ntasks; task += nwaves) {
+    if (task != wave) {
+      qrow = task * 32 + (lane & 31);
+      qrow_c = qrow < p.S ? qrow : p.S - 1;
+#pragma unroll
+      for (int s = 0; s < KS; ++s) qf[s] = gload8_nb<DP>(Qb, p.q_stride, qrow_c, 16 * s + 8 * hi, p.hd);
+    }
+    f32x16 accO[DB];
 #pragma unroll
     for (int d = 0; d < DB; ++d)
 #pragma unroll
-      for (int rq = 0; rq < 4; ++rq) {
-        const int col = d * 32 + 8 * rq + 4 * hi;
-        if (col < p.hd) {
-          bf16x4_bits o;
-#pragma unroll
-          for (int j = 0; j < 4; ++j) o[j] = f2bf_s(accO[d][4 * rq + j] * inv_l);
-          *reinterpret_cast<bf16x4_bits*>(Ob + col) = o;
-        }
-      }
-    if (hi == 0 && p.lse) p.lse[((int64_t)b * p.H + h) * p.S + qrow] = m_run * sl2 * LN2 + __logf(l_run);
+      for (int r = 0; r < 16; ++r) accO[d][r] = 0.f;
+    float m_run = -INFINITY, l_run = 0.f;
+    for (int t = 0; t < n_free; ++t)
+      fwd32_tile_math<DP, false>(Ks + t * BKV * KSTR, Vs + t * BKV * VSTR, qf, accO, m_run, l_run, t * BKV, p.S, 0, qrow, sl2, lane);
+    for (int t = n_free; t < ntiles; ++t)
+      fwd32_tile_math<DP, true>(Ks + t * BKV * KSTR, Vs + t * BKV * VSTR, qf, accO, m_run, l_run, t * BKV, p.S, 0, qrow, sl2, lane);
+    fwd32_finish<DP>(p, accO, m_run, l_run, b, h, qrow, sl2, hi);
   }
 }
 
@@ -444,6 +544,116 @@
     }
     *reinterpret_cast<bf16x4_bits*>(dst + col) = olo;
     *reinterpret_cast<bf16x4_bits*>(dst + half + col) = ohi;
+  }
+}
+
+template <int DP, bool MASK, bool BATCH>
+OVLA_DEV void dq_tile_math(const bf16_bits* Kt, const bf16_bits* Vt, const bf16x8_bits (&qf)[DP / 32], const bf16x8_bits (&dof)[DP / 32], f32x4 (&accQ)[DP / 16],
+                          float Lq, float Dq, int kbase, int kvlen, int causal, int qrow, float sl2, int lane) {
+  constexpr int KS = DP / 32, DT = DP / 16, STRIDE = DP + 16;
+  const int g = lane >> 4;
+#pragma unroll
+  for (int s2 = 0; s2 < 2; ++s2) {
+    f32x4 accS[2], accP[2];
+    if constexpr (BATCH) {
+      bf16x8_bits kfr[2][KS], vfr[2][KS];
+#pragma unroll
+      for (int nn = 0; nn < 2; ++nn)
+#pragma unroll
+        for (int s = 0; s < KS; ++s) {
+          kfr[nn][s] = row_frag(Kt, (2 * s2 + nn) * 16 + (lane & 15), 32 * s + 8 * g, STRIDE);
+          vfr[nn][s] = row_frag(Vt, (2 * s2 + nn) * 16 + (lane & 15), 32 * s + 8 * g, STRIDE);
+        }
+      __builtin_amdgcn_sched_barrier(0);
+#pragma unroll
+      for (int nn = 0; nn < 2; ++nn) {
+        accS[nn] = f32x4{0.f, 0.f, 0.f, 0.f};
+        accP[nn] = f32x4{0.f, 0.f, 0.f, 0.f};
+      }
+#pragma unroll
+      for (int s = 0; s < KS; ++s)
+#pragma unroll
+        for (int nn = 0; nn < 2; ++nn) {
+          accS[nn] = __builtin_amdgcn_mfma_f32_16x16x32_bf16(kfr[nn][s], qf[s], accS[nn], 0, 0, 0);
+          accP[nn] = __builtin_amdgcn_mfma_f32_16x16x32_bf16(vfr[nn][s], dof[s], accP[nn], 0, 0, 0);
+        }
+      __builtin_amdgcn_sched_barrier(0);
+    } else {
+#pragma unroll
+    for (int nn = 0; nn < 2; ++nn) {
+      const int nt = 2 * s2 + nn;
+      accS[nn] = f32x4{0.f, 0.f, 0.f, 0.f};
+      accP[nn] = f32x4{0.f, 0.f, 0.f, 0.f};
+#pragma unroll
+      for (int s = 0; s < KS; ++s) {
+        accS[nn] = __builtin_amdgcn_mfma_f32_16x16x32_bf16(row_frag(Kt, nt * 16 + (lane & 15), 32 * s + 8 * g, STRIDE), qf[s], accS[nn], 0, 0, 0);
+        accP[nn] = __builtin_amdgcn_mfma_f32_16x16x32_bf16(row_frag(Vt, nt * 16 + (lane & 15), 32 * s + 8 * g, STRIDE), dof[s], accP[nn], 0, 0, 0);
+      }
+    }
+    }
+    bf16x8_bits dsf;
+#pragma unroll
+    for (int nn = 0; nn < 2; ++nn)
+#pragma unroll
+      for (int j = 0; j < 4; ++j) {
+        float pv = __builtin_amdgcn_exp2f(accS[nn][j] * sl2 - Lq);
+        if constexpr (MASK) {
+          const int key = kbase + (2 * s2 + nn) * 16 + 4 * g + j;
+          const bool ok = key < kvlen && (!causal || key <= qrow);
+          pv = ok ? pv : 0.f;
+        }
+        dsf[4 * nn + j] = f2bf_s(pv * (accP[nn][j] - Dq));
+      }
+    if constexpr (BATCH) {
+      bf16x8_bits ktr[DT];
+#pragma unroll
+      for (int d = 0; d < DT; ++d) ktr[d] = tr_frag(Kt, 32 * s2, d * 16, STRIDE, lane);
+      __builtin_amdgcn_sched_barrier(0);
+#pragma unroll
+      for (int d = 0; d < DT; ++d) accQ[d] = __builtin_amdgcn_mfma_f32_16x16x32_bf16(ktr[d], dsf, accQ[d], 0, 0, 0);
+    } else {
+#pragma unroll
+    for (int d = 0; d < DT; ++d)
+      accQ[d] = __builtin_amdgcn_mfma_f32_16x16x32_bf16(tr_frag(Kt, 32 * s2, d * 16, STRIDE, lane), dsf, accQ[d], 0, 0, 0);
+    }
+  }
+}
+
+template <int KS>
+OVLA_DEV void dq_row_setup(const AttnParams& p, const bf16_bits* Qb, const bf16_bits* dOb, int b, int h, int qrow, int g,
+                          bf16x8_bits (&qf)[KS], bf16x8_bits (&dof)[KS], float& Lq, float& Dq) {
+  const int qrow_c = qrow < p.S ? qrow : p.S - 1;
+#pragma unroll
+  for (int s = 0; s < KS; ++s) {
+    qf[s] = gload8(Qb, p.q_stride, qrow_c, 32 * s + 8 * g, p.hd);
+    dof[s] = gload8(dOb, p.do_stride, qrow_c, 32 * s + 8 * g, p.hd);
+  }
+  const int64_t stat = ((int64_t)b * p.H + h) * p.S + qrow_c;
+  Lq = p.lse_in[stat] * LOG2E;
+  Dq = 0.f;
+  const bf16_bits* Ob = p.O + (int64_t)b * p.S * p.o_stride + (int64_t)h * p.hd;
+#pragma unroll
+  for (int s = 0; s < KS; ++s) {
+    const bf16x8_bits of = gload8(Ob, p.o_stride, qrow_c, 32 * s + 8 * g, p.hd);
+#pragma unroll
+    for (int j = 0; j < 8; ++j) Dq += bf2f((bf16_bits)of[j]) * bf2f((bf16_bits)dof[s][j]);
+  }
+  Dq += __shfl_xor(Dq, 16, 64);
+  Dq += __shfl_xor(Dq, 32, 64);
+  if (g == 0 && qrow < p.S) p.delta[stat] = Dq;
+}
+
+template <int DT>
+OVLA_DEV void grad_row_store(const f32x4 (&acc)[DT], float scale, bf16_bits* dst, int hd, int g) {
+#pragma unroll
+  for (int d = 0; d < DT; ++d) {
+    const int col = d * 16 + 4 * g;
+    if (col < hd) {
+      bf16x4_bits o;
+#pragma unroll
+      for (int j = 0; j < 4; ++j) o[j] = f2bf_s(acc[d][j] * scale);
+      *reinterpret_cast<bf16x4_bits*>(dst + col) = o;
+    }
   }
 }
 
@@ -462,7 +672,6 @@
     b = bh / p.H; h = bh - b * p.H; q0 = (wi - bh * nqb) * BQW;
   }
   const int qrow = q0 + wave * 16 + (lane & 15);
-  const int qrow_c = qrow < p.S ? qrow : p.S - 1;
   const int kvlen = p.kv_len ? p.kv_len[b] : p.S;
   int kv_end = kvlen < p.S ? kvlen : p.S;
   if (p.causal) kv_end = kv_end < (q0 + BQW) ? kv_end : (q0 + BQW);
@@ -474,26 +683,8 @@
   const bf16_bits* dOb = p.dO + (int64_t)b * p.S * p.do_stride + (int64_t)h * p.hd;
 
   bf16x8_bits qf[KS], dof[KS];
-#pragma unroll
-  for (int s = 0; s < KS; ++s) {
-    qf[s] = gload8(Qb, p.q_stride, qrow_c, 32 * s + 8 * g, p.hd);
-    dof[s] = gload8(dOb, p.do_stride, qrow_c, 32 * s + 8 * g, p.hd);
-  }
-  const int64_t stat = ((int64_t)b * p.H + h) * p.S + qrow_c;
-  const float Lq = p.lse_in[stat] * LOG2E;
-  float Dq = 0.f;
-  {
-    const bf16_bits* Ob = p.O + (int64_t)b * p.S * p.o_stride + (int64_t)h * p.hd;
-#pragma unroll
-    for (int s = 0; s < KS; ++s) {
-      const bf16x8_bits of = gload8(Ob, p.o_stride, qrow_c, 32 * s + 8 * g, p.hd);
-#pragma unroll
-      for (int j = 0; j < 8; ++j) Dq += bf2f((bf16_bits)of[j]) * bf2f((bf16_bits)dof[s][j]);
-    }
-    Dq += __shfl_xor(Dq, 16, 64);
-    Dq += __shfl_xor(Dq, 32, 64);
-    if (g == 0 && qrow < p.S) p.delta[stat] = Dq;
-  }
+  float Lq, Dq;
+  dq_row_setup<KS>(p, Qb, dOb, b, h, qrow, g, qf, dof, Lq, Dq);
   const float sl2 = p.scale * LOG2E;
 
   f32x4 accQ[DT];
@@ -516,72 +707,7 @@
     constexpr bool MASK = decltype(mask_tag)::value;
     const bf16_bits* Kt = Ks[t & 1];
     const bf16_bits* Vt = Vs[t & 1];
-    const int kbase = t * BKV;
-#pragma unroll
-    for (int s2 = 0; s2 < 2; ++s2) {
-      f32x4 accS[2], accP[2];
-      if constexpr (BATCH) {
-        bf16x8_bits kfr[2][KS], vfr[2][KS];
-#pragma unroll
-        for (int nn = 0; nn < 2; ++nn)
-#pragma unroll
-          for (int s = 0; s < KS; ++s) {
-            kfr[nn][s] = row_frag(Kt, (2 * s2 + nn) * 16 + (lane & 15), 32 * s + 8 * g, STRIDE);
-            vfr[nn][s] = row_frag(Vt, (2 * s2 + nn) * 16 + (lane & 15), 32 * s + 8 * g, STRIDE);
-          }
-        __builtin_amdgcn_sched_barrier(0);
-#pragma unroll
-        for (int nn = 0; nn < 2; ++nn) {
-          accS[nn] = f32x4{0.f, 0.f, 0.f, 0.f};
-          accP[nn] = f32x4{0.f, 0.f, 0.f, 0.f};
-        }
-#pragma unroll
-        for (int s = 0; s < KS; ++s)
-#pragma unroll
-          for (int nn = 0; nn < 2; ++nn) {
-            accS[nn] = __builtin_amdgcn_mfma_f32_16x16x32_bf16(kfr[nn][s], qf[s], accS[nn], 0, 0, 0);
-            accP[nn] = __builtin_amdgcn_mfma_f32_16x16x32_bf16(vfr[nn][s], dof[s], accP[nn], 0, 0, 0);
-          }
-        __builtin_amdgcn_sched_barrier(0);
-      } else {
-#pragma unroll
-      for (int nn = 0; nn < 2; ++nn) {
-        const int nt = 2 * s2 + nn;
-        accS[nn] = f32x4{0.f, 0.f, 0.f, 0.f};
-        accP[nn] = f32x4{0.f, 0.f, 0.f, 0.f};
-#pragma unroll
-        for (int s = 0; s < KS; ++s) {
-          accS[nn] = __builtin_amdgcn_mfma_f32_16x16x32_bf16(row_frag(Kt, nt * 16 + (lane & 15), 32 * s + 8 * g, STRIDE), qf[s], accS[nn], 0, 0, 0);
-          accP[nn] = __builtin_amdgcn_mfma_f32_16x16x32_bf16(row_frag(Vt, nt * 16 + (lane & 15), 32 * s + 8 * g, STRIDE), dof[s], accP[nn], 0, 0, 0);
-        }
-      }
-      }
-      bf16x8_bits dsf;
-#pragma unroll
-      for (int nn = 0; nn < 2; ++nn)
-#pragma unroll
-        for (int j = 0; j < 4; ++j) {
-          float pv = __builtin_amdgcn_exp2f(accS[nn][j] * sl2 - Lq);
-          if constexpr (MASK) {
-            const int key = kbase + (2 * s2 + nn) * 16 + 4 * g + j;
-            const bool ok = key < kvlen && (!p.causal || key <= qrow);
-            pv = ok ? pv : 0.f;
-          }
-          dsf[4 * nn + j] = f2bf_s(pv * (accP[nn][j] - Dq));
-        }
-      if constexpr (BATCH) {
-        bf16x8_bits ktr[DT];
-#pragma unroll
-        for (int d = 0; d < DT; ++d) ktr[d] = tr_frag(Kt, 32 * s2, d * 16, STRIDE, lane);
-        __builtin_amdgcn_sched_barrier(0);
-#pragma unroll
-        for (int d = 0; d < DT; ++d) accQ[d] = __builtin_amdgcn_mfma_f32_16x16x32_bf16(ktr[d], dsf, accQ[d], 0, 0, 0);
-      } else {
-#pragma unroll
-      for (int d = 0; d < DT; ++d)
-        accQ[d] = __builtin_amdgcn_mfma_f32_16x16x32_bf16(tr_frag(Kt, 32 * s2, d * 16, STRIDE, lane), dsf, accQ[d], 0, 0, 0);
-      }
-    }
+    dq_tile_math<DP, MASK, BATCH>(Kt, Vt, qf, dof, accQ, Lq, Dq, t * BKV, kvlen, p.causal, qrow, sl2, lane);
     if (t + 1 < ntiles) {
       kst.store(Ks[(t + 1) & 1], tid);
       vst.store(Vs[(t + 1) & 1], tid);
@@ -602,20 +728,60 @@
     if (p.rope_cos) {
       inverse_rope_store<DT>(accQ, p.scale, dQb, p.hd, qrow, g, p.rope_cos, p.rope_sin);
     } else {
-#pragma unroll
-      for (int d = 0; d < DT; ++d) {
-        const int col = d * 16 + 4 * g;
-        if (col < p.hd) {
-          bf16x4_bits o;
-#pragma unroll
-          for (int j = 0; j < 4; ++j) o[j] = f2bf_s(accQ[d][j] * p.scale);
-          *reinterpret_cast<bf16x4_bits*>(dQb + col) = o;
+      grad_row_store<DT>(accQ, p.scale, dQb, p.hd, g);
+    }
+  }
+}
+
+
+template <int DP, bool MASK>
+OVLA_DEV void dkv_tile_math(const bf16_bits* Qt, const bf16_bits* dOt, const float* Lt, const float* Dt, const bf16x8_bits (&kf)[DP / 32], const bf16x8_bits (&vf)[DP / 32],
+                           f32x4 (&accK)[DP / 16], f32x4 (&accV)[DP / 16], int qbase, int S, bool key_ok, int causal, int krow, float sl2, int lane) {
+  constexpr int KS = DP / 32, DT = DP / 16, STRIDE = DP + 16;
+  const int g = lane >> 4;
+#pragma unroll
+  for (int s2 = 0; s2 < 2; ++s2) {
+    f32x4 accS[2], accP[2];
+#pragma unroll
+    for (int mm = 0; mm < 2; ++mm) {
+      const int mt = 2 * s2 + mm;
+      accS[mm] = f32x4{0.f, 0.f, 0.f, 0.f};
+      accP[mm] = f32x4{0.f, 0.f, 0.f, 0.f};
+#pragma unroll
+      for (int s = 0; s < KS; ++s) {
+        accS[mm] = __builtin_amdgcn_mfma_f32_16x16x32_bf16(row_frag(Qt, mt * 16 + (lane & 15), 32 * s + 8 * g, STRIDE), kf[s], accS[mm], 0, 0, 0);
+        accP[mm] = __builtin_amdgcn_mfma_f32_16x16x32_bf16(row_frag(dOt, mt * 16 + (lane & 15), 32 * s + 8 * g, STRIDE), vf[s], accP[mm], 0, 0, 0);
+      }
+    }
+#pragma unroll
+    for (int mm = 0; mm < 2; ++mm)
+#pragma unroll
+      for (int j = 0; j < 4; ++j) {
+        const int ql = (2 * s2 + mm) * 16 + 4 * g + j;
+        float pv = __builtin_amdgcn_exp2f(accS[mm][j] * sl2 - Lt[ql]);
+        if constexpr (MASK) {
+          const int q = qbase + ql;
+          const bool ok = key_ok && q < S && (!causal || krow <= q);
+          pv = ok ? pv : 0.f;
         }
-      }
-    }
-  }
-}
-
+        accS[mm][j] = pv;
+        accP[mm][j] = pv * (accP[mm][j] - Dt[ql]);
+      }
+    bf16x8_bits pf, dsf;
+#pragma unroll
+    for (int j = 0; j < 4; ++j) {
+      pf[j] = f2bf_s(accS[0][j]);
+      pf[4 + j] = f2bf_s(accS[1][j]);
+      dsf[j] = f2bf_s(accP[0][j]);
+      dsf[4 + j] = f2bf_s(accP[1][j]);
+    }
+#pragma unroll
+    for (int d = 0; d < DT; ++d) {
+      accV[d] = __builtin_amdgcn_mfma_f32_16x16x32_bf16(tr_frag(dOt, 32 * s2, d * 16, STRIDE, lane), pf, accV[d], 0, 0, 0);
+      accK[d] = __builtin_amdgcn_mfma_f32_16x16x32_bf16(tr_frag(Qt, 32 * s2, d * 16, STRIDE, lane), dsf, accK[d], 0, 0, 0);
+    }
+  }
+}
 
 template <int DP, int NW>
 __global__ __launch_bounds__(64 * NW, 2) void attn_bwd_dkv_kernel(const AttnParams p) {
@@ -694,49 +860,7 @@
     const bf16_bits* dOt = dOs[buf];
     const float* Lt = Ls[buf];
     const float* Dt = Ds[buf];
-    const int qbase = qt * BQ;
-#pragma unroll
-    for (int s2 = 0; s2 < 2; ++s2) {
-      f32x4 accS[2], accP[2];
-#pragma unroll
-      for (int mm = 0; mm < 2; ++mm) {
-        const int mt = 2 * s2 + mm;
-        accS[mm] = f32x4{0.f, 0.f, 0.f, 0.f};
-        accP[mm] = f32x4{0.f, 0.f, 0.f, 0.f};
-#pragma unroll
-        for (int s = 0; s < KS; ++s) {
-          accS[mm] = __builtin_amdgcn_mfma_f32_16x16x32_bf16(row_frag(Qt, mt * 16 + (lane & 15), 32 * s + 8 * g, STRIDE), kf[s], accS[mm], 0, 0, 0);
-          accP[mm] = __builtin_amdgcn_mfma_f32_16x16x32_bf16(row_frag(dOt, mt * 16 + (lane & 15), 32 * s + 8 * g, STRIDE), vf[s], accP[mm], 0, 0, 0);
-        }
-      }
-#pragma unroll
-      for (int mm = 0; mm < 2; ++mm)
-#pragma unroll
-        for (int j = 0; j < 4; ++j) {
-          const int ql = (2 * s2 + mm) * 16 + 4 * g + j;
-          float pv = __builtin_amdgcn_exp2f(accS[mm][j] * sl2 - Lt[ql]);
-          if constexpr (MASK) {
-            const int q = qbase + ql;
-            const bool ok = key_ok && q < p.S && (!p.causal || krow <= q);
-            pv = ok ? pv : 0.f;
-          }
-          accS[mm][j] = pv;
-          accP[mm][j] = pv * (accP[mm][j] - Dt[ql]);
-        }
-      bf16x8_bits pf, dsf;
-#pragma unroll
-      for (int j = 0; j < 4; ++j) {
-        pf[j] = f2bf_s(accS[0][j]);
-        pf[4 + j] = f2bf_s(accS[1][j]);
-        dsf[j] = f2bf_s(accP[0][j]);
-        dsf[4 + j] = f2bf_s(accP[1][j]);
-      }
-#pragma unroll
-      for (int d = 0; d < DT; ++d) {
-        accV[d] = __builtin_amdgcn_mfma_f32_16x16x32_bf16(tr_frag(dOt, 32 * s2, d * 16, STRIDE, lane), pf, accV[d], 0, 0, 0);
-        accK[d] = __builtin_amdgcn_mfma_f32_16x16x32_bf16(tr_frag(Qt, 32 * s2, d * 16, STRIDE, lane), dsf, accK[d], 0, 0, 0);
-      }
-    }
+    dkv_tile_math<DP, MASK>(Qt, dOt, Lt, Dt, kf, vf, accK, accV, qt * BQ, p.S, key_ok, p.causal, krow, sl2, lane);
     if (qt + 1 < nq) {
       store_tile(buf ^ 1);
       if (qt + 2 < nq) load_tile(qt + 2);
@@ -770,6 +894,81 @@
   }
 }
 
+constexpr int RES_BWD_WAVES_MAX = 16;
+
+template <int DP>
+__global__ __launch_bounds__(64 * RES_BWD_WAVES_MAX) void attn_bwd_resident_kernel(const AttnParams p) {
+  constexpr int KS = DP / 32, DT = DP / 16, STRIDE = DP + 16;
+  extern __shared__ __attribute__((aligned(16))) char res_smem[];
+  const int ntiles = (p.S + BKV - 1) / BKV, rows = ntiles * BKV;
+  float* Ls = reinterpret_cast<float*>(res_smem);
+  float* Ds = Ls + rows;
+  bf16_bits* As = reinterpret_cast<bf16_bits*>(Ds + rows);
+  bf16_bits* Bs = As + rows * STRIDE;
+
+  const int tid = threadIdx.x, lane = tid & 63, wave = tid >> 6, g = lane >> 4, nwaves = blockDim.x >> 6;
+  const int bh = blockIdx.x, b = bh / p.H, h = bh - b * p.H;
+  const bf16_bits* Qb = p.Q + (int64_t)b * p.S * p.q_stride + (int64_t)h * p.hd;
+  const bf16_bits* Kb = p.K + (int64_t)b * p.S * p.k_stride + (int64_t)h * p.hd;
+  const bf16_bits* Vb = p.V + (int64_t)b * p.S * p.v_stride + (int64_t)h * p.hd;
+  const bf16_bits* dOb = p.dO + (int64_t)b * p.S * p.do_stride + (int64_t)h * p.hd;
+  const float* lse_b = p.lse_in + ((int64_t)b * p.H + h) * p.S;
+  const float sl2 = p.scale * LOG2E;
+  const int ntasks = (p.S + 15) / 16, n_free = p.S / BKV;
+
+  stage_resident<DP, STRIDE>(As, Kb, p.k_stride, ntiles, p.S - 1, p.hd, tid, blockDim.x);
+  stage_resident<DP, STRIDE>(Bs, Vb, p.v_stride, ntiles, p.S - 1, p.hd, tid, blockDim.x);
+  for (int r = tid; r < rows; r += blockDim.x) Ls[r] = lse_b[r < p.S ? r : p.S - 1] * LOG2E;
+  __syncthreads();
+  for (int task = wave; task < ntasks; task += nwaves) {
+    const int qrow = task * 16 + (lane & 15);
+    bf16x8_bits qf[KS], dof[KS];
+    float Lq, Dq;
+    dq_row_setup<KS>(p, Qb, dOb, b, h, qrow, g, qf, dof, Lq, Dq);
+    if (g == 0) Ds[qrow] = Dq;
+    f32x4 accQ[DT];
+#pragma unroll
+    for (int d = 0; d < DT; ++d) accQ[d] = f32x4{0.f, 0.f, 0.f, 0.f};
+    for (int t = 0; t < n_free; ++t)
+      dq_tile_math<DP, false, false>(As + t * BKV * STRIDE, Bs + t * BKV * STRIDE, qf, dof, accQ, Lq, Dq, t * BKV, p.S, 0, qrow, sl2, lane);
+    for (int t = n_free; t < ntiles; ++t)
+      dq_tile_math<DP, true, false>(As + t * BKV * STRIDE, Bs + t * BKV * STRIDE, qf, dof, accQ, Lq, Dq, t * BKV, p.S, 0, qrow, sl2, lane);
+    if (qrow < p.S) grad_row_store<DT>(accQ, p.scale, p.dQ + ((int64_t)b * p.S + qrow) * p.dq_stride + (int64_t)h * p.hd, p.hd, g);
+  }
+  __syncthreads();
+
+  for (int r = ntasks * 16 + tid; r < rows; r += blockDim.x) Ds[r] = Ds[p.S - 1];
+  stage_resident<DP, STRIDE>(As, Qb, p.q_stride, ntiles, p.S - 1, p.hd, tid, blockDim.x);
+  stage_resident<DP, STRIDE>(Bs, dOb, p.do_stride, ntiles, p.S - 1, p.hd, tid, blockDim.x);
+  __syncthreads();
+  for (int task = wave; task < ntasks; task += nwaves) {
+    const int k0 = task * 16, krow = k0 + (lane & 15);
+    const int krow_c = krow < p.S ? krow : p.S - 1;
+    bf16x8_bits kf[KS], vf[KS];
+#pragma unroll
+    for (int s = 0; s < KS; ++s) {
+      kf[s] = gload8(Kb, p.k_stride, krow_c, 32 * s + 8 * g, p.hd);
+      vf[s] = gload8(Vb, p.v_stride, krow_c, 32 * s + 8 * g, p.hd);
+    }
+    f32x4 accK[DT], accV[DT];
+#pragma unroll
+    for (int d = 0; d < DT; ++d) {
+      accK[d] = f32x4{0.f, 0.f, 0.f, 0.f};
+      accV[d] = f32x4{0.f, 0.f, 0.f, 0.f};
+    }
+    const bool key_ok = krow < p.S;
+    const int n_freeq = (k0 + 16 <= p.S) ? n_free : 0;
+    for (int qt = 0; qt < n_freeq; ++qt)
+      dkv_tile_math<DP, false>(As + qt * BQ * STRIDE, Bs + qt * BQ * STRIDE, Ls + qt * BQ, Ds + qt * BQ, kf, vf, accK, accV, qt * BQ, p.S, key_ok, 0, krow, sl2, lane);
+    for (int qt = n_freeq; qt < ntiles; ++qt)
+      dkv_tile_math<DP, true>(As + qt * BQ * STRIDE, Bs + qt * BQ * STRIDE, Ls + qt * BQ, Ds + qt * BQ, kf, vf, accK, accV, qt * BQ, p.S, key_ok, 0, krow, sl2, lane);
+    if (krow < p.S) {
+      grad_row_store<DT>(accK, p.scale, p.dK + ((int64_t)b * p.S + krow) * p.dk_stride + (int64_t)h * p.hd, p.hd, g);
+      grad_row_store<DT>(accV, 1.0f, p.dV + ((int64_t)b * p.S + krow) * p.dv_stride + (int64_t)h * p.hd, p.hd, g);
+    }
+  }
+}
+
 int check_common(int B, int H, int S, int hd, const char* who) {
   if (!(B > 0 && H > 0 && S > 0)) {
     ovla_set_error("%s: empty problem B=%d H=%d S=%d", who, B, H, S);
@@ -784,7 +983,58 @@
 
 inline bool stride_ok(int64_t s) { return (s % 8) == 0; }
 
-}
+constexpr int RES_MIN_BH_64_FWD = 192, RES_MIN_BH_64_BWD = 128, RES_MIN_BH_72_FWD = 0, RES_MIN_BH_72_BWD = 160;
+std::atomic<int64_t> g_resident_launches{0};
+
+int resident_min_bh(int hd, bool backward) {
+  static const int forced = []() {
+    const char* e = getenv("OVLA_ATTN_RESIDENT");
+    if (!e || !e[0]) return -1;
+    const int n = atoi(e);
+    return n > 0 ? n : 0;
+  }();
+  if (!(hd == 64 || hd == 72)) return INT32_MAX;
+  const int v = forced >= 0 ? forced : hd == 64 ? (backward ? RES_MIN_BH_64_BWD : RES_MIN_BH_64_FWD) : (backward ? RES_MIN_BH_72_BWD : RES_MIN_BH_72_FWD);
+  return v > 0 ? v : INT32_MAX;
+}
+
+bool resident_shape(int hd, int S, bool masked, int64_t bh, bool backward) {
+  return (hd == 64 || hd == 72) && !masked && S > 64 && S <= resident_max_s(hd) && bh >= resident_min_bh(hd, backward);
+}
+
+template <typename Kernel>
+int allow_full_lds(Kernel kernel, const char* who) {
+  static std::atomic<uint64_t> done{0};
+  int dev = 0;
+  hipError_t e = hipGetDevice(&dev);
+  const uint64_t bit = 1ull << (dev & 63);
+  if (e == hipSuccess && (done.load(std::memory_order_acquire) & bit)) return OVLA_OK;
+  if (e == hipSuccess) e = hipFuncSetAttribute(reinterpret_cast<const void*>(kernel), hipFuncAttributeMaxDynamicSharedMemorySize, RES_LDS_BYTES);
+  if (e != hipSuccess) {
+    ovla_set_error("%s: cannot allow %d bytes of LDS per workgroup: %s", who, RES_LDS_BYTES, hipGetErrorString(e));
+    return OVLA_ELAUNCH;
+  }
+  done.fetch_or(bit, std::memory_order_release);
+  return OVLA_OK;
+}
+
+template <typename Kernel>
+int launch_resident(Kernel kernel, const AttnParams& p, int waves, bool backward, hipStream_t stream, const char* who) {
+  if (int rc = allow_full_lds(kernel, who)) return rc;
+  hipLaunchKernelGGL(kernel, dim3((unsigned)(p.B * p.H)), dim3(64 * waves), (size_t)resident_lds_bytes(p.hd, p.S, backward), stream, p);
+  g_resident_launches.fetch_add(1, std::memory_order_relaxed);
+  return OVLA_OK;
+}
+
+}
+
+extern "C" int32_t ovla_attn_resident_max_s(int32_t head_dim) { return resident_max_s(head_dim); }
+extern "C" int64_t ovla_attn_resident_lds_bytes(int32_t head_dim, int32_t S, int32_t backward) {
+  if (!(S > 0 && S <= resident_max_s(head_dim))) return -1;
+  return resident_lds_bytes(head_dim, S, backward != 0);
+}
+extern "C" int32_t ovla_attn_resident_min_bh(int32_t head_dim, int32_t backward) { return resident_min_bh(head_dim, backward != 0); }
+extern "C" int64_t ovla_attn_resident_launches(void) { return g_resident_launches.load(std::memory_order_relaxed); }
 
 extern "C" int ovla_attn_fwd(const ovla_attn_fwd_args* a, void* stream_) {
   hipStream_t stream = (hipStream_t)stream_;
@@ -800,7 +1050,12 @@
   static const bool fwd32 = []() { const char* e = getenv("OVLA_ATTN_FWD32"); return !(e && e[0] == '0'); }();
   static const bool xcd_map = []() { const char* e = getenv("OVLA_ATTN_XCD"); return !(e && e[0] == '0'); }();
   p.xcd_map = xcd_map ? 1 : 0;
-  if (fwd32 && a->S > 64) {
+  if (fwd32 && resident_shape(a->head_dim, a->S, a->kv_len || a->causal, (int64_t)a->B * a->H, false)) {
+    const int tasks = cdiv(a->S, 32);
+    if (int rc = a->head_dim == 64 ? launch_resident(attn_fwd_resident_kernel<64, 10>, p, tasks < 10 ? tasks : 10, false, stream, "ovla_attn_fwd")
+                                   : launch_resident(attn_fwd_resident_kernel<96, 8>, p, tasks < 8 ? tasks : 8, false, stream, "ovla_attn_fwd"))
+      return rc;
+  } else if (fwd32 && a->S > 64) {
     const dim3 grid((unsigned)(cdiv(a->S, 128) * a->H * a->B));
     switch (a->head_dim) {
       case 64: hipLaunchKernelGGL((attn_fwd32_kernel<64>), grid, dim3(256), 0, stream, p); break;
@@ -850,6 +1105,14 @@
   const dim3 grid = xcd_map ? dim3((unsigned)(cdiv(a->S, BQ) * a->H * a->B)) : dim3(cdiv(a->S, BQ), a->H, a->B);
   const dim3 grid_kv4 = grid;
   const dim3 grid_kv8 = xcd_map ? dim3((unsigned)(cdiv(a->S, 128) * a->H * a->B)) : dim3(cdiv(a->S, 128), a->H, a->B);
+  if (resident_shape(a->head_dim, a->S, a->kv_len || a->causal || a->rope_cos, (int64_t)a->B * a->H, true)) {
+    const int tasks = cdiv(a->S, 16), waves = tasks < RES_BWD_WAVES_MAX ? tasks : RES_BWD_WAVES_MAX;
+    if (int rc = a->head_dim == 64 ? launch_resident(attn_bwd_resident_kernel<64>, p, waves, true, stream, "ovla_attn_bwd")
+                                   : launch_resident(attn_bwd_resident_kernel<96>, p, waves, true, stream, "ovla_attn_bwd"))
+      return rc;
+    OVLA_CHECK_LAUNCH("ovla_attn_bwd");
+    return OVLA_OK;
+  }
   switch (a->head_dim) {
     case 64:
       hipLaunchKernelGGL((attn_bwd_dq_kernel<64, 4>), grid, dim3(256), 0, stream, p);
```

Measured after the change: 49.33 samples/s (median of 2 runs). No clear change (-0.0%).
